# alexmeli100/pbrt-rust

Hardware: AMD Instinct MI355X
Metric: Msamples/s (camera rays x spp) at 1920x1080 (higher is better)
Workload: dtype f32

## Files before the change

include/mi355pt.h:

```cpp
#ifndef MI355PT_H
#define MI355PT_H

#include <stdint.h>

#ifdef __cplusplus
extern "C" {
#endif

typedef enum PtStatus {
    PT_OK = 0,
    PT_ERR_INVALID_ARG = 1,
    PT_ERR_NO_DEVICE = 2,
    PT_ERR_HIP = 3,
    PT_ERR_UNSUPPORTED = 4,
    PT_ERR_SOBOL_DIMENSIONS = 5,
    PT_ERR_STACK_OVERFLOW = 6,
    PT_ERR_OUT_OF_MEMORY = 7,
    PT_ERR_PROBE_CHAIN = 8
} PtStatus;


enum {
    PT_TRI_REVERSE_ORIENTATION = 1u << 0,
    PT_TRI_SWAPS_HANDEDNESS    = 1u << 1,
// ... 257 lines not shown
typedef struct PtCounters {
    uint64_t camera_rays;
    uint64_t intersect_tests;
    uint64_t shadow_tests;
    uint64_t bvh_nodes_visited;
    uint64_t triangle_tests;
    uint64_t sphere_tests;
    uint64_t zero_radiance_paths_num, zero_radiance_paths_den;
    uint64_t path_length_hist[16];
    uint64_t sanitized_nan, sanitized_negative, sanitized_infinite;
    uint64_t film_splats;
    uint64_t wavefront_stages;
    uint64_t reference_asserts;
} PtCounters;

typedef struct PtKernelStat {
    char name[32];
    uint64_t launches;
    double total_ms;
    uint64_t items;
    uint64_t bvh_nodes;
    uint64_t triangle_tests;
    char kernel[48];
} PtKernelStat;

typedef struct pt_scene pt_scene;
typedef struct pt_multi_scene pt_multi_scene;


int pt_init(int device_ordinal);
int pt_device_count(int *n_devices);
const char *pt_last_error(void);
int pt_set_trace_exact(int exact);

int pt_scene_create(const PtSceneDesc *desc, pt_scene **out_scene);
void pt_scene_destroy(pt_scene *scene);

int pt_scene_bvh_info(const pt_scene *scene, uint32_t *n_nodes, uint32_t *n_prims);
int pt_scene_bvh_read(const pt_scene *scene, PtBVHNode *nodes, uint32_t *ordered_prims);

int pt_render(pt_scene *scene, const PtRenderParams *params, float *film_xyzw, int film_is_device);
int pt_render_samples(pt_scene *scene, const PtRenderParams *params, uint32_t first_sample, uint32_t n_samples, float *film_xyzw, int film_is_device);
int pt_pass_size(pt_scene *scene, const PtRenderParams *params, uint32_t *spp_per_pass);

int pt_film_resolve(const float *film_xyzw, uint32_t n_pixels, float scale, float *rgb_out);

int pt_film_resolve_device(pt_scene *scene, const float *film_xyzw_dev, uint32_t n_pixels, float scale, float *rgb_dev, uint8_t *srgb8_dev);
int pt_film_halves_error(pt_scene *scene, const float *film_a_dev, const float *film_b_dev, uint32_t width, uint32_t height,
                         float *tile_error_dev, float *mean_error_host, float *max_tile_error_host);

int pt_tile_grid(const PtRenderParams *params, uint32_t *ntx, uint32_t *nty);
int pt_render_tiles(pt_scene *scene, const PtRenderParams *params, uint32_t first_sample, uint32_t n_samples,
                    const uint32_t *tiles, uint32_t n_tiles, float *film_xyzw, int film_is_device);
int pt_tiles_select(pt_scene *scene, const PtRenderParams *params, const float *tile_error_dev, float threshold,
                    const uint32_t *candidates, uint32_t n_candidates, uint32_t *tiles_out, uint32_t *n_out);

int pt_multi_scene_create(const PtSceneDesc *desc, const int *device_ordinals, uint32_t n_devices, pt_multi_scene **out_scene);
void pt_multi_scene_destroy(pt_multi_scene *scene);
int pt_multi_render(pt_multi_scene *scene, const PtRenderParams *params, float *film_xyzw, int film_is_device);
int pt_multi_render_samples(pt_multi_scene *scene, const PtRenderParams *params, uint32_t first_sample, uint32_t n_samples, float *film_xyzw, int film_is_device);
int pt_multi_get_counters(const pt_multi_scene *scene, PtCounters *out);
int pt_multi_get_kernel_stats(const pt_multi_scene *scene, uint32_t replica, PtKernelStat *out, uint32_t max_entries, uint32_t *n_out);
int pt_multi_get_timing(const pt_multi_scene *scene, double *merge_ms, double *render_ms, double *copy_ms, uint32_t max_replicas);
int pt_multi_get_create_timing(const pt_multi_scene *scene, double *wall_ms, double *replica_ms, uint32_t max_replicas);
enum { PT_PEER_SAME_DEVICE = 0, PT_PEER_ENABLED = 1, PT_PEER_STAGED = 2 };
int pt_multi_get_peer_access(const pt_multi_scene *scene, int *peer, uint32_t max_replicas);
void pt_multi_tile_shard(uint32_t tile_rank, uint32_t tile_world, uint32_t replica, uint32_t n_replicas, uint32_t *rank_out, uint32_t *world_out);

int pt_get_counters(const pt_scene *scene, PtCounters *out);
int pt_get_kernel_stats(const pt_scene *scene, PtKernelStat *out, uint32_t max_entries, uint32_t *n_out);

int pt_trace_closest(pt_scene *scene, uint32_t n, const float *origins, const float *dirs,
                     const float *tmax, uint32_t *out_prim, float *out_t, float *out_b);
int pt_trace_any(pt_scene *scene, uint32_t n, const float *origins, const float *dirs,
                 const float *tmax, uint8_t *out_hit);
int pt_sobol_samples(const int32_t sample_bounds[4], uint32_t n, const int32_t *pixel_xy,
                     const uint32_t *sample_num, uint32_t n_dims, float *out, uint64_t *out_index);
int pt_halton_samples(const int32_t sample_bounds[4], uint32_t sample_at_pixel_center, uint32_t n, const int32_t *pixel_xy,
                      const uint32_t *sample_num, uint32_t n_dims, float *out, uint64_t *out_index);
int pt_camera_rays(const PtRenderParams *params, uint32_t n, const float *camera_samples,
                   float *out_origins, float *out_dirs);
int pt_dist1d_sample(const float *func, uint32_t n, int discrete, uint32_t n_u, const float *u,
                     float *out_x, float *out_pdf, int32_t *out_offset);

#ifdef __cplusplus
}
#endif
#endif
```

pbrt-rust_amd/_abi.py:

```python
import ctypes as C

PT_OK = 0
PT_ERR_INVALID_ARG, PT_ERR_NO_DEVICE, PT_ERR_HIP, PT_ERR_UNSUPPORTED = 1, 2, 3, 4
PT_ERR_SOBOL_DIMENSIONS, PT_ERR_STACK_OVERFLOW, PT_ERR_OUT_OF_MEMORY, PT_ERR_PROBE_CHAIN = 5, 6, 7, 8

PT_TRI_REVERSE_ORIENTATION = 1
PT_TRI_SWAPS_HANDEDNESS = 2
PT_TRI_HAS_N = 4
PT_TRI_HAS_S = 8
PT_TRI_HAS_UV = 16

PT_SHAPE_TRIANGLE, PT_SHAPE_SPHERE = 0, 1
PT_NONE = 0xFFFFFFFF

PT_MAT_MATTE, PT_MAT_MIRROR, PT_MAT_GLASS, PT_MAT_PLASTIC, PT_MAT_METAL, PT_MAT_UBER, PT_MAT_SUBSTRATE, PT_MAT_SUBSURFACE, PT_MAT_TRANSLUCENT, PT_MAT_MIX, PT_MAT_DISNEY = range(11)
(PT_DS_METALLIC, PT_DS_SPECULARTINT, PT_DS_ANISOTROPIC, PT_DS_SHEEN, PT_DS_SHEENTINT, PT_DS_CLEARCOAT, PT_DS_CLEARCOATGLOSS, PT_DS_SPECTRANS,
 PT_DS_FLATNESS, PT_DS_DIFFTRANS) = range(10)
PT_LIGHT_DIFFUSE_AREA, PT_LIGHT_DISTANT, PT_LIGHT_POINT, PT_LIGHT_INFINITE, PT_LIGHT_SPOT = range(5)
PT_LS_UNIFORM, PT_LS_POWER, PT_LS_SPATIAL, PT_LS_SPATIAL_EAGER, PT_LS_SPATIAL_LAZY = range(5)
PT_SPLIT_SAH, PT_SPLIT_HLBVH = range(2)
PT_SAMPLER_SOBOL, PT_SAMPLER_HALTON = range(2)
PT_INTEGRATOR_PATH, PT_INTEGRATOR_VOLPATH = range(2)
PT_QUADRIC_SPHERE, PT_QUADRIC_DISK = range(2)

# ... 74 lines not shown
                ("rhoeff", fp), ("profile_cdf", fp)]


class PtSceneDesc(C.Structure):
    _fields_ = [("n_vertices", u32), ("P", fp), ("N", fp), ("S", fp), ("UV", fp),
                ("n_triangles", u32), ("indices", u32p), ("tri_flags", u8p),
                ("n_spheres", u32), ("spheres", C.POINTER(PtSphere)),
                ("n_prims", u32), ("prim_shape", u32p), ("prim_material", u32p), ("prim_light", u32p),
                ("n_materials", u32), ("materials", C.POINTER(PtMaterial)),
                ("n_lights", u32), ("lights", C.POINTER(PtLight)),
                ("env_width", u32), ("env_height", u32), ("env_texels", fp), ("env_importance", fp), ("env_power_lookup", f32 * 3),
                ("max_node_prims", u32), ("n_nodes", u32), ("nodes", C.POINTER(PtBVHNode)), ("ordered_prims", u32p),
                ("n_objects", u32), ("objects", C.POINTER(PtObject)), ("n_instances", u32), ("instances", C.POINTER(PtInstance)),
                ("n_top", u32), ("top_refs", u32p), ("n_bssrdf_tables", u32), ("bssrdf_tables", C.POINTER(PtBSSRDFTable)),
                ("n_textures", u32), ("textures", C.POINTER(PtTexture)), ("tri_alpha", i32p), ("tri_shadow_alpha", i32p), ("n_images", u32), ("images", C.POINTER(PtImage)), ("ewa_weight_lut", fp), ("n_media", u32), ("media", C.POINTER(PtMedium)), ("prim_medium_inside", u32p), ("prim_medium_outside", u32p), ("split_method", u32)]


class PtRenderParams(C.Structure):
    _fields_ = [("full_resolution", i32 * 2), ("cropped_pixel_bounds", i32 * 4), ("filter_radius", f32 * 2),
                ("filter_table", f32 * 256), ("max_sample_luminance", f32), ("scale", f32),
                ("spp", u32), ("sample_bounds", i32 * 4),
                ("raster_to_camera", f32 * 16), ("camera_to_world", f32 * 16), ("lens_radius", f32),
                ("focal_distance", f32), ("shutter_open", f32), ("shutter_close", f32),
                ("max_depth", u32), ("rr_threshold", f32), ("pixel_bounds", i32 * 4), ("light_strategy", u32),
                ("tile_rank", u32), ("tile_world", u32), ("spp_per_pass", u32), ("profile", u32), ("sampler_type", u32), ("sample_at_pixel_center", u32), ("integrator", u32), ("camera_medium", u32)]


class PtCounters(C.Structure):
    _fields_ = [("camera_rays", u64), ("intersect_tests", u64), ("shadow_tests", u64), ("bvh_nodes_visited", u64),
                ("triangle_tests", u64), ("sphere_tests", u64), ("zero_radiance_paths_num", u64),
                ("zero_radiance_paths_den", u64), ("path_length_hist", u64 * 16), ("sanitized_nan", u64),
                ("sanitized_negative", u64), ("sanitized_infinite", u64), ("film_splats", u64),
                ("wavefront_stages", u64), ("reference_asserts", u64)]

    def as_dict(self):
        d = {}
        for name, _ in self._fields_:
            v = getattr(self, name)
            d[name] = list(v) if hasattr(v, "__len__") else int(v)
        return d


class PtKernelStat(C.Structure):
    _fields_ = [("name", C.c_char * 32), ("launches", u64), ("total_ms", C.c_double), ("items", u64), ("bvh_nodes", u64), ("triangle_tests", u64), ("kernel", C.c_char * 48)]


VP = C.c_void_p
ENTRY_POINTS = {
    "pt_init": (C.c_int, [C.c_int]),
    "pt_last_error": (C.c_char_p, []),
    "pt_scene_create": (C.c_int, [C.POINTER(PtSceneDesc), C.POINTER(VP)]),
    "pt_scene_destroy": (None, [VP]),
    "pt_scene_bvh_info": (C.c_int, [VP, u32p, u32p]),
    "pt_scene_bvh_read": (C.c_int, [VP, C.POINTER(PtBVHNode), u32p]),
    "pt_render": (C.c_int, [VP, C.POINTER(PtRenderParams), VP, C.c_int]),
    "pt_render_samples": (C.c_int, [VP, C.POINTER(PtRenderParams), u32, u32, VP, C.c_int]),
    "pt_pass_size": (C.c_int, [VP, C.POINTER(PtRenderParams), u32p]),
    "pt_tile_grid": (C.c_int, [C.POINTER(PtRenderParams), u32p, u32p]),
    "pt_render_tiles": (C.c_int, [VP, C.POINTER(PtRenderParams), u32, u32, u32p, u32, VP, C.c_int]),
    "pt_tiles_select": (C.c_int, [VP, C.POINTER(PtRenderParams), VP, f32, u32p, u32, u32p, u32p]),
    "pt_film_resolve": (C.c_int, [fp, u32, f32, fp]),
    "pt_film_resolve_device": (C.c_int, [VP, VP, u32, f32, VP, VP]),
    "pt_film_halves_error": (C.c_int, [VP, VP, VP, u32, u32, VP, fp, fp]),
    "pt_device_count": (C.c_int, [C.POINTER(C.c_int)]),
    "pt_set_trace_exact": (C.c_int, [C.c_int]),
    "pt_multi_scene_create": (C.c_int, [C.POINTER(PtSceneDesc), C.POINTER(C.c_int), u32, C.POINTER(VP)]),
    "pt_multi_scene_destroy": (None, [VP]),
    "pt_multi_render": (C.c_int, [VP, C.POINTER(PtRenderParams), VP, C.c_int]),
    "pt_multi_render_samples": (C.c_int, [VP, C.POINTER(PtRenderParams), u32, u32, VP, C.c_int]),
    "pt_multi_get_counters": (C.c_int, [VP, C.POINTER(PtCounters)]),
    "pt_multi_get_kernel_stats": (C.c_int, [VP, u32, C.POINTER(PtKernelStat), u32, u32p]),
    "pt_multi_get_timing": (C.c_int, [VP, C.POINTER(C.c_double), C.POINTER(C.c_double), C.POINTER(C.c_double), u32]),
    "pt_multi_get_peer_access": (C.c_int, [VP, C.POINTER(C.c_int), u32]),
    "pt_multi_get_create_timing": (C.c_int, [VP, C.POINTER(C.c_double), C.POINTER(C.c_double), u32]),
    "pt_multi_tile_shard": (None, [u32, u32, u32, u32, u32p, u32p]),
    "pt_get_counters": (C.c_int, [VP, C.POINTER(PtCounters)]),
    "pt_get_kernel_stats": (C.c_int, [VP, C.POINTER(PtKernelStat), u32, u32p]),
    "pt_trace_closest": (C.c_int, [VP, u32, fp, fp, fp, u32p, fp, fp]),
    "pt_trace_any": (C.c_int, [VP, u32, fp, fp, fp, u8p]),
    "pt_sobol_samples": (C.c_int, [i32p, u32, i32p, u32p, u32, fp, u64p]),
    "pt_halton_samples": (C.c_int, [i32p, u32, u32, i32p, u32p, u32, fp, u64p]),
    "pt_camera_rays": (C.c_int, [C.POINTER(PtRenderParams), u32, fp, fp, fp]),
    "pt_dist1d_sample": (C.c_int, [fp, u32, C.c_int, u32, fp, fp, fp, i32p]),
}


def bind(lib, table=ENTRY_POINTS, strict=True):
    for name, (res, args) in table.items():
        fn = getattr(lib, name, None)
        if fn is None:
            if strict:
                raise AttributeError(f"{name}: symbol declared in " + ("include/mi355pt.h" if table is ENTRY_POINTS else "its C header") + " is missing from the library")
            continue
        fn.restype = res
        fn.argtypes = args
    return lib
```

pbrt-rust_amd/csrc/kern_aux.h:

```cpp
#pragma once
#include "kern_shade_common.h"
#include "kern_film.h"
__global__ __launch_bounds__(256) void k_medium_route(DeviceScene s, RenderConst rc, SobolTables tabs, PathSoA ps, const uint32_t *queue, const uint32_t *count_ptr,
                                                     uint32_t *class_count, uint32_t *c0, uint32_t *c1, uint32_t *c2, uint32_t *c3, uint32_t *c4, uint32_t *c5, uint32_t *error) {
    __shared__ LdsQueue<1024> q0, q1, q2, q3, q4, q5;
    lq_init(q0); lq_init(q1); lq_init(q2); lq_init(q3); lq_init(q4); lq_init(q5);
    __syncthreads();
    const uint32_t count = *count_ptr;
    const uint32_t rounded = (count + 255u) & ~255u;
    for (uint32_t qi = blockIdx.x * blockDim.x + threadIdx.x; qi < rounded; qi += gridDim.x * blockDim.x) {
        const bool valid = qi < count;
        uint32_t pid = 0, cls = (uint32_t)kMissClass;
        if (valid) {
            pid = queue[qi];
            const uint32_t hp = ps.hit_prim(pid);
            cls = class_general((ps.hit_pflags(pid) >> kTpClassShift) & kTpClassMask);
            if (cls == (uint32_t)kSpecClass) cls = 1u;
            const uint32_t med = ps.medium(pid);
            if (med != PT_NONE) {
                uint32_t meta = ps.meta(pid);
                Sampler smp = make_sampler(tabs, nullptr, 0u, ps.sobol_index(pid), meta & 0xffffu, rc.halton.enabled != 0);
                const V3 rd(ps.dx(pid), ps.dy(pid), ps.dz(pid));
                bool sampled; float t;
                RGB w(1.0f);
// ... 25 lines not shown
        lq_flush_nosync(q4, class_count + 4, c4, 256u, false); lq_flush_nosync(q5, class_count + 5, c5, 256u, false);
        __syncthreads();
    }
    lq_flush_nosync(q0, class_count + 0, c0, 0u, true); lq_flush_nosync(q1, class_count + 1, c1, 0u, true);
    lq_flush_nosync(q2, class_count + 2, c2, 0u, true); lq_flush_nosync(q3, class_count + 3, c3, 0u, true);
    lq_flush_nosync(q4, class_count + 4, c4, 0u, true); lq_flush_nosync(q5, class_count + 5, c5, 0u, true);
}

__global__ __launch_bounds__(256) void k_shade_medium(DeviceScene s, RenderConst rc, SobolTables tabs, LightGrid grid, PathSoA ps, ShadeJob job) {
    constexpr uint32_t LDS_DIMS = 56u;
    __shared__ uint32_t s_sobol[LDS_DIMS * kSobolNibWords];
    __shared__ VertexQueues<1024, false, true> s_q;
    __shared__ uint32_t s_hist[16];
    s_q.init();
    hist_init(s_hist);
    PT_PROF_BEGIN
    sobol_stage_lds(s_sobol, tabs.nib, LDS_DIMS, threadIdx.x, blockDim.x);
    __syncthreads();
    const uint32_t count = *job.count;
    const uint32_t rounded = (count + 255u) & ~255u;
    unsigned long long zero_num = 0, n_valid = 0, n_bytes = 0;
    uint32_t n_assert = 0;
    for (uint32_t qi = blockIdx.x * blockDim.x + threadIdx.x; qi < rounded; qi += gridDim.x * blockDim.x) {
        const bool valid = qi < count;
        bool push_ext = false, push_resolve = false, push_shadow = false, push_mis = false, push_self = false;
        int finished_bounces = -1;
        uint32_t pid = 0;
        if (valid) {
            n_valid++;
            pid = job.queue[qi];
            const uint32_t meta = ps.meta(pid);
            uint32_t flags = meta >> 24, bounces = (meta >> 16) & 0xffu;
            Sampler smp = make_sampler(tabs, s_sobol, LDS_DIMS, ps.sobol_index(pid), meta & 0xffffu, rc.halton.enabled != 0);
            RGB L(ps.L_r(pid), ps.L_g(pid), ps.L_b(pid));
            RGB beta(ps.beta_r(pid), ps.beta_g(pid), ps.beta_b(pid));
            const bool stage_b = (flags & PF_STAGE_B) != 0u;
            if (stage_b) smp.load_window();
            if (stage_b && s.has_shells) { if (!vol_chain_step<true>(s, ps, pid, flags, smp, push_shadow, push_mis, n_bytes)) resolve_pending<true, true>(s, ps, pid, flags, L, zero_num, n_assert, n_bytes PT_PROF_PASS, nullptr); }
            else resolve_pending<true, true>(s, ps, pid, flags, L, zero_num, n_assert, n_bytes PT_PROF_PASS, stage_b ? &smp : nullptr);
            flags &= ~(PF_CAMERA_RAY | PF_STAGE_B);
            bool terminated = bounces >= rc.max_depth;
            if (!terminated) {
                if (!stage_b) smp.load_window();
                const V3 ro(ps.ox(pid), ps.oy(pid), ps.oz(pid)), rd(ps.dx(pid), ps.dy(pid), ps.dz(pid));
                const uint32_t med = ps.medium(pid);
                SurfaceInteraction si;
                si.p = ro + rd * ps.hit_t(pid); si.wo = -rd; si.n = V3(0.0f, 0.0f, 0.0f); si.sh_n = V3(0.0f, 0.0f, 0.0f); si.p_error = V3(0.0f, 0.0f, 0.0f);
                IData it; it.p = si.p; it.p_error = V3(0.0f, 0.0f, 0.0f); it.n = V3(0.0f, 0.0f, 0.0f);
                const PhaseBsdf phase{s.media[med].g, si.wo};
                bool defer = false;
                if (!stage_b) {
                    if (!nee_vertex<true, PhaseBsdf, true, true>(s, grid, ps, pid, smp, si, it, phase, beta, flags, push_shadow, push_mis, n_bytes PT_PROF_PASS, MedIface{med, med})) L = L + beta * RGB(0.0f);
                }
                defer = (s.has_grid != 0u || s.has_shells != 0u) && (push_shadow || push_mis);
                if (defer) { flags |= PF_STAGE_B; push_self = true; }
                else {
                V3 wi;
                hg_sample_p(phase.g, si.wo, wi, smp.get_2d());
                flags &= ~PF_SPECULAR;
                if (russian_roulette(rc, smp, beta, ps.etascale(pid), bounces, n_assert)) terminated = true;
                else {
                    bounces += 1;
                    ps.ox(pid) = si.p.x; ps.oy(pid) = si.p.y; ps.oz(pid) = si.p.z;
                    ps.dx(pid) = wi.x; ps.dy(pid) = wi.y; ps.dz(pid) = wi.z;
                    push_ext = true;
                }
                }
            }
            if (terminated) {
                if (flags & (PF_PEND_SHADOW | PF_PEND_MIS)) { flags |= PF_DEAD; push_resolve = true; }
                else finished_bounces = (int)bounces;
            }
            store_vertex(ps, pid, L, beta, smp, bounces, flags, job.error);
        }
        s_q.push(job, pid, push_ext, push_resolve, push_shadow, push_mis, push_self);
        if (finished_bounces >= 0) hist_add(s_hist, (uint32_t)finished_bounces);
        s_q.flush(job, 256u, false);
    }
    s_q.flush(job, 0u, true);
    vertex_epilogue(s_hist, job.counters, &job.counters->shade_items[kMediumClass], &job.counters->shade_bytes[kMediumClass], n_valid, n_bytes, n_assert);
    (void)zero_num;
}

template <bool SPH, bool VOL>
__global__ __launch_bounds__(256, PT_MISS_WAVES) void k_shade_miss(DeviceScene s, RenderConst rc, PathSoA ps, ShadeJob job) {
    __shared__ uint32_t s_hist[16];
    hist_init(s_hist);
    PT_PROF_BEGIN
    __syncthreads();
    const uint32_t count = *job.count;
    unsigned long long zero_num = 0, n_valid = 0, n_bytes = 0;
    uint32_t n_assert = 0;
    for (uint32_t qi = blockIdx.x * blockDim.x + threadIdx.x; qi < count; qi += gridDim.x * blockDim.x) {
        n_valid++;
        n_bytes += 4 + 32 +  16 + 4;
        const uint32_t pid = job.queue[qi];
        float4 *cq = reinterpret_cast<float4 *>(ps.core) + 4 * (size_t)pid;
        const float4 c0 = cq[0], c1 = cq[1];
        const uint32_t meta = __float_as_uint(c1.w);
        uint32_t flags = meta >> 24; const uint32_t bounces = (meta >> 16) & 0xffu;
        RGB L(c0.x, c0.y, c0.z);
        resolve_pending<SPH, VOL>(s, ps, pid, flags, L, zero_num, n_assert, n_bytes PT_PROF_PASS);
        if (!(flags & PF_DEAD) && (bounces == 0 || (flags & PF_SPECULAR)) && s.n_infinite > 0) {
            n_bytes += 32;
            const RGB beta(c1.x, c1.y, c1.z);
            const float4 *rq = reinterpret_cast<const float4 *>(ps.ray) + 2 * (size_t)pid;
            const float4 r0 = rq[0], r1 = rq[1];
            const V3 rd(r0.w, r1.x, r1.y);
            add_escaped_le(s, rd, beta, L);
        }
        cq[0] = make_float4(L.r, L.g, L.b, c0.w);
        ps.meta(pid) = (meta & 0x00ffffffu) | ((flags & ~PF_CAMERA_RAY) << 24);
        hist_add(s_hist, bounces);
    }
    __syncthreads();
    counter_add(&job.counters->zero_num, zero_num);
    vertex_epilogue(s_hist, job.counters, &job.counters->shade_items[kMissClass], &job.counters->shade_bytes[kMissClass], n_valid, n_bytes, n_assert);
    (void)rc;
}

template <bool SPH>
__global__ __launch_bounds__(256, PT_FILM_WAVES) void k_film_final(DeviceScene s, RenderConst rc, PathSoA ps, const float *filter_table, float *film_rgbw, DevCounters *counters) {
    __shared__ uint32_t s_hist[16];
    hist_init(s_hist);
    __syncthreads();
    PT_PROF_BEGIN
    unsigned long long zero_num = 0, n_final = 0, n_bytes = 0;
    uint32_t n_assert = 0;
    film_slot(rc, ps, filter_table, film_rgbw, counters, [&](uint32_t pid, RGB &L) {
        const float4 c1 = reinterpret_cast<const float4 *>(ps.core)[4 * (size_t)pid + 1];
        const uint32_t meta = __float_as_uint(c1.w);
        uint32_t flags = meta >> 24; const uint32_t bounces = (meta >> 16) & 0xffu;
        const bool pend = (flags & (PF_PEND_SHADOW | PF_PEND_MIS)) != 0u;
        const bool escaped = !(flags & (PF_DEAD | PF_FINISHED));
        if (!pend && !escaped) return;
        n_final++; n_bytes += 32 + 4;
        resolve_pending<SPH, false, true>(s, ps, pid, flags, L, zero_num, n_assert, n_bytes PT_PROF_PASS);
        if (escaped && (bounces == 0 || (flags & PF_SPECULAR)) && s.n_infinite > 0) {
            n_bytes += 32;
            const RGB beta(c1.x, c1.y, c1.z);
            const float4 *rq = reinterpret_cast<const float4 *>(ps.ray) + 2 * (size_t)pid;
            const float4 r0 = rq[0], r1 = rq[1];
            const V3 rd(r0.w, r1.x, r1.y);
            add_escaped_le(s, rd, beta, L);
        }
        hist_add(s_hist, bounces);
    });
    __syncthreads();
    counter_add(&counters->zero_num, zero_num);
    vertex_epilogue(s_hist, counters, &counters->shade_items[kMissClass], &counters->shade_bytes[kMissClass], n_final, n_bytes, n_assert);
}
```

pbrt-rust_amd/csrc/kern_decl.h:

```cpp
#pragma once
#include "kern_common.h"

template <int ANY, int MODE, bool PROBE, int QUADK> __global__ void k_trace(DeviceScene s, TraceJob job);
template <int MAXL, int MODE, int DIFF> __global__ void k_shade(DeviceScene s, RenderConst rc, SobolTables tabs, LightGrid grid, PathSoA ps, ShadeJob job);
template <bool SPH, bool VOL> __global__ void k_shade_miss(DeviceScene s, RenderConst rc, PathSoA ps, ShadeJob job);
template <bool SPH, bool VOL> __global__ void k_bssrdf(DeviceScene s, RenderConst rc, SobolTables tabs, LightGrid grid, PathSoA ps, BssrdfJob job);
__global__ void k_medium_route(DeviceScene s, RenderConst rc, SobolTables tabs, PathSoA ps, const uint32_t *queue, const uint32_t *count_ptr,
                               uint32_t *class_count, uint32_t *c0, uint32_t *c1, uint32_t *c2, uint32_t *c3, uint32_t *c4, uint32_t *c5, uint32_t *error);
__global__ void k_shade_medium(DeviceScene s, RenderConst rc, SobolTables tabs, LightGrid grid, PathSoA ps, ShadeJob job);
__global__ void k_build_packets(DeviceScene s, const uint32_t *ordered, uint32_t n_refs, TriPacket *out);
__global__ void k_mark_leaf_ends(TriPacket *leaf, const uint32_t *last_index, uint32_t n);
__global__ void k_light_area(DeviceScene s, const uint32_t *head, float *area, float4 *rec);
template <int NQ, int CAP> __global__ void k_route(DeviceScene s, const uint32_t *queue, const uint32_t *count_ptr, PathSoA ps, uint32_t *class_count, RouteJob rj);
__global__ void k_generate(RenderConst rc, SobolTables tabs, PathSoA ps, uint32_t *q_ext, uint32_t *q_ext_count, DevCounters *counters);
__global__ void k_film(RenderConst rc, PathSoA ps, const float *filter_table, float *film_rgbw, DevCounters *counters);
template <bool SPH> __global__ void k_film_final(DeviceScene s, RenderConst rc, PathSoA ps, const float *filter_table, float *film_rgbw, DevCounters *counters);
__global__ void k_film_finish(const float *film_rgbw, float *film_xyzw, uint32_t npix);
__global__ void k_film_resolve(const float4 *film_xyzw, uint32_t n_pixels, float scale, float *rgb, uint8_t *srgb8, int packed);
__global__ void k_film_halves_error(const float4 *film_a, const float4 *film_b, uint32_t width, uint32_t height, uint32_t ntx, float *tile_sum, float *tile_err);
__global__ void k_film_error_reduce(const float *tile_sum, const float *tile_err, uint32_t n_tiles, float n_pixels, float *out);
__global__ void k_tiles_select(RenderConst rc, const float *tile_err, float threshold, const uint32_t *candidates, uint32_t n_candidates, uint32_t *out);
__global__ void k_film_sum(FilmSumArgs a, float4 *dst, int accumulate, size_t n_quads);
__global__ void k_light_grid_contrib(DeviceScene s, uint32_t nvx, uint32_t nvy, uint32_t nvz, float *func, const uint32_t *cells, size_t n_cells, size_t stride);
__global__ void k_light_grid_finish(uint32_t n_lights, size_t ncell, float *func, float *cdf, float *func_int, const uint32_t *cells, size_t stride, unsigned long long *cell_ptr);
template <bool SPH> __global__ void k_light_touch(DeviceScene s, LightGrid g, PathSoA ps, const uint32_t *queue, const uint32_t *count_ptr, uint32_t kind, uint32_t max_depth, uint32_t *req_flag, uint32_t *req_list, uint32_t *req_count);
__global__ void k_halton_samples(SobolTables tabs, HaltonParams hp, uint32_t n, const int32_t *pixel_xy, const uint32_t *sample_num,
                                 uint32_t n_dims, float *out, uint64_t *out_index);
__global__ void k_sobol_samples(SobolTables tabs, SobolParams sp, uint32_t n, const int32_t *pixel_xy, const uint32_t *sample_num,
                                uint32_t n_dims, float *out, uint64_t *out_index);
__global__ void k_camera_rays(RenderConst rc, uint32_t n, const float *cs, float *out_o, float *out_d);
__global__ void k_dist1d_sample(const float *func, const float *cdf, float func_int, int n, int discrete, uint32_t n_u, const float *u, float *out_x, float *out_pdf, int32_t *out_off);
```

pbrt-rust_amd/csrc/kern_misc.h:

```cpp
#pragma once
#include "kern_common.h"
#include "kern_film.h"
__global__ void k_build_packets(DeviceScene s, const uint32_t *ordered, uint32_t n_refs, TriPacket *out) {
    uint32_t i = blockIdx.x * blockDim.x + threadIdx.x;
    if (i >= n_refs) return;
    uint32_t prim = ordered[i];
    TriPacket p;
    if (prim & PT_TOP_INSTANCE) {
        p.x[0] = p.x[1] = p.x[2] = p.y[0] = p.y[1] = p.y[2] = p.z[0] = p.z[1] = p.z[2] = 0.0f;
        p.prim = PT_NONE; p.shape = prim & ~PT_TOP_INSTANCE; p.flags = TP_INSTANCE;
        out[i] = p;
        return;
    }
    uint32_t shape = s.prim_shape[prim];
    p.prim = prim; p.shape = shape; p.flags = 0;
    const uint32_t mat = s.prim_material[prim];
    const uint32_t hi = ((mat == PT_NONE ? 0u : (uint32_t)s.mat_class[mat]) << kTpClassShift) | ((mat == PT_NONE || mat >= kTpMatNone ? kTpMatNone : mat) << kTpMatShift);
    if ((shape >> 30) == PT_SHAPE_TRIANGLE) {
        uint32_t tri = shape & 0x3fffffffu;
        uint32_t i0 = s.indices[3 * tri], i1 = s.indices[3 * tri + 1], i2 = s.indices[3 * tri + 2];
        V3 p0 = ld3(s.P, i0), p1 = ld3(s.P, i1), p2 = ld3(s.P, i2);
        P2 uv[3]; tri_uvs(s, tri, i0, i1, i2, uv);
        V3 dpdu, dpdv;
        bool ok = tri_partials(p0, p1, p2, uv, dpdu, dpdv);
        p.x[0] = p0.x; p.x[1] = p1.x; p.x[2] = p2.x; p.y[0] = p0.y; p.y[1] = p1.y; p.y[2] = p2.y; p.z[0] = p0.z; p.z[1] = p1.z; p.z[2] = p2.z;
        p.flags = (uint32_t)s.tri_flags[tri] | (ok ? 0u : (uint32_t)TP_BOGUS) | hi;
        if ((s.tri_alpha && s.tri_alpha[tri] >= 0) || (s.tri_shadow_alpha && s.tri_shadow_alpha[tri] >= 0)) p.flags |= TP_ALPHA;
    } else {
        p.x[0] = p.x[1] = p.x[2] = p.y[0] = p.y[1] = p.y[2] = p.z[0] = p.z[1] = p.z[2] = 0.0f;
        p.flags = TP_SPHERE | hi;
    }
    out[i] = p;
}

__global__ void k_mark_leaf_ends(TriPacket *leaf, const uint32_t *last_index, uint32_t n) {
    uint32_t i = blockIdx.x * blockDim.x + threadIdx.x;
    if (i < n) leaf[last_index[i]].flags |= TP_LAST;
}

__global__ void k_light_area(DeviceScene s, const uint32_t *head, float *area, float4 *rec) {
    uint32_t i = blockIdx.x * blockDim.x + threadIdx.x;
    if (i >= s.n_lights) return;
    float a = 0.0f;
    const PtLight &L = s.lights[i];
    float4 r0 = make_float4(0.0f, 0.0f, 0.0f, __uint_as_float(head[i])), r1 = make_float4(0.0f, 0.0f, 0.0f, 0.0f), r2 = r1, r4 = r1, r5 = r1;
    if (L.type == PT_LIGHT_DIFFUSE_AREA) {
        uint32_t shape = s.prim_shape[L.prim];
        if ((shape >> 30) == PT_SHAPE_TRIANGLE) {
            uint32_t tri = shape & 0x3fffffffu;
            const V3 p0 = ld3(s.P, s.indices[3 * tri]), p1 = ld3(s.P, s.indices[3 * tri + 1]), p2 = ld3(s.P, s.indices[3 * tri + 2]);
            a = tri_area(p0, p1, p2);
            const uint32_t fl = s.tri_flags[tri];
            const bool flip = ((fl & PT_TRI_REVERSE_ORIENTATION) != 0) != ((fl & PT_TRI_SWAPS_HANDEDNESS) != 0);
            V3 ns = normalize(cross(p1 - p0, p2 - p0));
            if (!(fl & PT_TRI_HAS_N) && flip) ns = ns * -1.0f;
            V3 np = normalize(cross(p0 - p2, p1 - p2));
            if (flip) np = -np;
            P2 uv[3]; tri_uvs(s, tri, s.indices[3 * tri], s.indices[3 * tri + 1], s.indices[3 * tri + 2], uv);
            V3 dpdu, dpdv;
            const bool degenerate = !tri_partials(p0, p1, p2, uv, dpdu, dpdv);
            r4 = make_float4(ns.x, ns.y, ns.z, 1.0f / a); r5 = make_float4(np.x, np.y, np.z, 0.0f);
            r0 = make_float4(p0.x, p0.y, p0.z, __uint_as_float(fl | kLrecValid | (degenerate ? kLrecDegenerate : 0u) | head[i]));
            r1 = make_float4(p1.x, p1.y, p1.z, __uint_as_float(tri)); r2 = make_float4(p2.x, p2.y, p2.z, a);
        } else {
            const PtSphere &S = s.spheres[shape & 0x3fffffffu];
            a = S.kind == PT_QUADRIC_DISK ? S.phi_max * 0.5f * (S.radius * S.radius - S.inner_radius * S.inner_radius)
                                          : S.phi_max * S.radius * (S.z_max - S.z_min);
        }
    }
    area[i] = a;
    float4 *r = rec + 6 * (size_t)i;
    r[0] = r0; r[1] = r1; r[2] = r2; r[3] = make_float4(L.L[0], L.L[1], L.L[2], __uint_as_float(L.two_sided)); r[4] = r4; r[5] = r5;
}
template <int NQ, int CAP>
__global__ __launch_bounds__(256) void k_route(DeviceScene s, const uint32_t *queue, const uint32_t *count_ptr, PathSoA ps, uint32_t *class_count, RouteJob rj) {
    __shared__ LdsQueue<CAP> q[NQ];
#pragma unroll
    for (int k = 0; k < NQ; ++k) lq_init(q[k]);
    __syncthreads();
    const uint32_t count = *count_ptr;
    const uint32_t rounded = (count + 255u) & ~255u;
    for (uint32_t qi = blockIdx.x * blockDim.x + threadIdx.x; qi < rounded; qi += gridDim.x * blockDim.x) {
        const bool valid = qi < count;
        uint32_t pid = 0, cls = (uint32_t)kMissClass;
        if (valid) {
            pid = queue[qi];
            cls = (ps.hit_pflags(pid) >> kTpClassShift) & kTpClassMask;
        }
        const uint32_t slot = (uint32_t)(rj.slot_map >> (4u * cls)) & 15u;
        if (valid && slot == 15u && cls != rj.drop_cls) atomicMax(rj.error, (uint32_t)PT_ERR_UNSUPPORTED);
#pragma unroll
        for (int k = 0; k < NQ; ++k) if ((uint32_t)k < rj.n_slots) lq_push(q[k], pid, valid && slot == (uint32_t)k);
        __syncthreads();
#pragma unroll
        for (int k = 0; k < NQ; ++k) if ((uint32_t)k < rj.n_slots) lq_flush_nosync(q[k], class_count + rj.cls_of_slot[k], rj.buf[k], 256u, false);
        __syncthreads();
    }
#pragma unroll
    for (int k = 0; k < NQ; ++k) if ((uint32_t)k < rj.n_slots) lq_flush_nosync(q[k], class_count + rj.cls_of_slot[k], rj.buf[k], 0u, true);
}
PT_DEV void camera_ray(const RenderConst &rc, float pfx, float pfy, float time_u, P2 plens_u, V3 &o, V3 &d) {
    V3 pcamera = xf_point(rc.raster_to_camera, V3(pfx, pfy, 0.0f));
    V3 ro(0.0f, 0.0f, 0.0f), rd = normalize(pcamera);
    if (rc.lens_radius > 0.0f) {
        P2 dsk = concentric_sample_disk(plens_u);
        float lx = dsk.x * rc.lens_radius, ly = dsk.y * rc.lens_radius;
        float ft = rc.focal_distance / rd.z;
        V3 pfocus = ro + rd * ft;
        ro = V3(lx, ly, 0.0f);
        rd = normalize(pfocus - ro);
    }
    (void)time_u;
    V3 oerr;
    V3 ow = xf_point_err(rc.camera_to_world, ro, oerr);
    V3 dw = xf_vector(rc.camera_to_world, rd);
    float l2 = length_squared(dw);
    if (l2 > 0.0f) { float dt = dot(vabs(dw), oerr) / l2; ow = ow + dw * dt; }
    o = ow; d = dw;
}

constexpr int kGenPlane = 257;
struct GenStage { float4 core[4 * kGenPlane]; float4 ray[2 * kGenPlane]; uint32_t alive[256]; };
PT_DEV void stage_path(GenStage &g, uint32_t t, float pfx, float pfy, V3 o, V3 d, uint64_t index, uint32_t medium) {
    g.core[0 * kGenPlane + t] = make_float4(0.0f, 0.0f, 0.0f, 1.0f);
    g.core[1 * kGenPlane + t] = make_float4(1.0f, 1.0f, 1.0f, __uint_as_float(5u | (PF_CAMERA_RAY << 24)));
    g.core[2 * kGenPlane + t] = make_float4(__uint_as_float((uint32_t)index), __uint_as_float((uint32_t)(index >> 32)), pfx, pfy);
    g.core[3 * kGenPlane + t] = make_float4(__uint_as_float(medium), __uint_as_float(PT_NONE), 0.0f, 0.0f);
    g.ray[0 * kGenPlane + t] = make_float4(o.x, o.y, o.z, d.x); g.ray[1 * kGenPlane + t] = make_float4(d.y, d.z, 0.0f, 0.0f);
}
PT_DEV void flush_paths(const GenStage &g, const PathSoA &ps, uint32_t pid0, uint32_t t) {
    float4 *core = reinterpret_cast<float4 *>(ps.core) + 4 * (size_t)pid0, *ray = reinterpret_cast<float4 *>(ps.ray) + 2 * (size_t)pid0;
#pragma unroll
    for (uint32_t j = 0; j < 4; ++j) { const uint32_t gq = j * 256u + t, p = gq >> 2, q = gq & 3u; if (g.alive[p]) core[gq] = g.core[q * kGenPlane + p]; }
#pragma unroll
    for (uint32_t j = 0; j < 2; ++j) { const uint32_t gq = j * 256u + t, p = gq >> 1, q = gq & 1u; if (g.alive[p]) ray[gq] = g.ray[q * kGenPlane + p]; }
}

__global__ __launch_bounds__(256) void k_generate(RenderConst rc, SobolTables tabs, PathSoA ps, uint32_t *q_ext, uint32_t *q_ext_count, DevCounters *counters) {
    constexpr uint32_t kVdcNibbles = 13;
    __shared__ uint32_t s_nib[kSobolNibbles * 5 * 16];
    __shared__ uint64_t s_vdc[2 * kVdcNibbles * 16];
    __shared__ LdsQueue<1024> s_q;
    __shared__ GenStage s_gen;
    lq_init(s_q);
    const uint32_t m = (uint32_t)rc.sobol.log2_resolution;
    sobol_stage_lds(s_nib, tabs.nib, 5u, threadIdx.x, blockDim.x);
    if (m > 0) for (uint32_t i = threadIdx.x; i < 2 * kVdcNibbles * 16; i += blockDim.x) {
        const uint32_t which = i / (kVdcNibbles * 16), e = i - which * (kVdcNibbles * 16), j = e >> 4, n = e & 15u;
        const uint64_t *col = (which ? tabs.vdc_inv : tabs.vdc) + (m - 1) * 52 + 4 * j;
        uint64_t v = 0;
        for (uint32_t b = 0; b < 4; ++b) if (n & (1u << b)) v ^= col[b];
        s_vdc[i] = v;
    }
    __syncthreads();
    const uint32_t total = rc.n_pix_slots * rc.s_count;
    const uint32_t stride = gridDim.x * blockDim.x;
    const uint32_t rounded = (total + 255u) & ~255u;
    unsigned long long n_alive = 0;
    for (uint32_t pid = blockIdx.x * blockDim.x + threadIdx.x; pid < rounded; pid += stride) {
        bool alive = false;
        if (pid < total) {
            const uint32_t slot = pid % rc.n_pix_slots, sl = pid / rc.n_pix_slots;
            int32_t px, py;
            if (slot_to_pixel(rc, slot, px, py)) {
                const uint64_t sample = rc.s_begin + sl;
                if (rc.halton.enabled) {
                    const uint64_t index = halton_index_for_sample(rc.halton, px, py, sample);
                    const float fx = halton_sample_dimension(tabs, rc.halton, index, 0u), fy = halton_sample_dimension(tabs, rc.halton, index, 1u);
                    const float pfx = (float)px + fx, pfy = (float)py + fy;
                    const float tm = halton_sample_dimension(tabs, rc.halton, index, 2u);
                    const P2 pl(halton_sample_dimension(tabs, rc.halton, index, 3u), halton_sample_dimension(tabs, rc.halton, index, 4u));
                    V3 o, d;
                    camera_ray(rc, pfx, pfy, tm, pl, o, d);
                    stage_path(s_gen, threadIdx.x, pfx, pfy, o, d, index, rc.volpath ? rc.camera_medium : PT_NONE);
                    alive = true;
                } else {
                uint64_t index = 0;
                if (m != 0) {
                    index = sample << (m << 1);
                    uint64_t delta = 0;
                    for (uint64_t f = sample, j = 0; f != 0; f >>= 4, ++j) delta ^= s_vdc[j * 16 + (f & 15u)];
                    uint64_t b = ((uint64_t)((uint32_t)(px - rc.sobol.sb_min[0]) << m) | (uint64_t)(uint32_t)(py - rc.sobol.sb_min[1])) ^ delta;
// ... 158 lines not shown
```

pbrt-rust_amd/csrc/kern_shade_common.h:

```cpp
#pragma once
#include "kern_common.h"

#ifdef PT_REGION_PROFILE
struct Prof { long long *t; int *r; unsigned long long *acc; };
#define PT_PROF_BEGIN __shared__ long long s_pt[4]; __shared__ int s_pr[4]; __shared__ unsigned long long s_pacc[64]; \
    if (threadIdx.x < 64) s_pacc[threadIdx.x] = 0; \
    if (threadIdx.x < 4) { s_pt[threadIdx.x] = clock64(); s_pr[threadIdx.x] = 15; } \
    Prof prof{s_pt, s_pr, s_pacc};
#define PT_PROF_END(counters) do { PT_T(14); __syncthreads(); \
    if (threadIdx.x < 16) atomicAdd(&(counters)->regions[threadIdx.x], prof.acc[threadIdx.x] + prof.acc[16 + threadIdx.x] + prof.acc[32 + threadIdx.x] + prof.acc[48 + threadIdx.x]); } while (0)
#define PT_T(k) do { if ((int)__lane_id() == __ffsll((unsigned long long)__ballot(1)) - 1) { const long long _n = clock64(); const int _w = threadIdx.x >> 6; \
    prof.acc[_w * 16 + prof.r[_w]] += (unsigned long long)(_n - prof.t[_w]); prof.t[_w] = _n; prof.r[_w] = (k); } } while (0)
#define PT_PROF_ARG , Prof prof
#define PT_PROF_PASS , prof
#else
#define PT_T(k) do {} while (0)
#define PT_PROF_BEGIN
#define PT_PROF_END(counters) do {} while (0)
#define PT_PROF_ARG
#define PT_PROF_PASS
#endif

template <bool SPH, bool VOL = false, bool EARLY = false> PT_DEV void resolve_pending(const DeviceScene &s, const PathSoA &ps, uint32_t pid, uint32_t &flags, RGB &L,
                                                unsigned long long &zero_num, uint32_t &n_assert, unsigned long long &n_bytes PT_PROF_ARG, Sampler *smp = nullptr) {
// ... 44 lines not shown
            }
        }
        if (!lrad.is_black()) {
            RGB f(m3.x, m3.y, m3.z);
            if (VOL && !tr_done) {
                const uint32_t mm = ps.mis_medium(pid);
                if (mm != PT_NONE) Tr = Tr * medium_tr(s.media[mm], mp != PT_NONE ? m3.w : PT_INF, wi);
            }
            Ld = Ld + f * lrad * Tr * m1.z / m1.w;
        }
    }
    RGB nb(n3.x, n3.y, n3.z);
    RGB Ldb = nb * (Ld / n2.w);
    if (!VOL && Ldb.is_black() && !(flags & PF_NEE_UNCOUNTED)) zero_num++;
    if (!VOL && !(flags & PF_NEE_UNCOUNTED) && !(Ldb.y() >= 0.0f)) n_assert++;
    L = L + Ldb;
    flags &= ~(PF_PEND_SHADOW | PF_PEND_MIS | PF_NEE_UNCOUNTED);
}

template <bool SPH> PT_DEV bool vol_chain_step(const DeviceScene &s, const PathSoA &ps, uint32_t pid, uint32_t flags, Sampler &smp, bool &push_shadow, bool &push_mis,
                                              unsigned long long &n_bytes) {
    float4 *nq = reinterpret_cast<float4 *>(ps.nee) + 4 * (size_t)pid;
    float4 *mq = reinterpret_cast<float4 *>(ps.mis) + 4 * (size_t)pid;
    float4 *xq = reinterpret_cast<float4 *>(ps.ext) + 8 * (size_t)pid;
    if ((flags & PF_PEND_SHADOW) && __float_as_uint(nq[1].z) != 1u) {
        const float4 n0 = nq[0], n1 = nq[1], n2 = nq[2], n3 = nq[3], h0 = xq[4], h1 = xq[5];
        n_bytes += 64 + 32;
        const uint32_t prim = __float_as_uint(h0.x), sm = __float_as_uint(n3.w);
        const bool hit = prim != PT_NONE;
        const V3 so(n0.x, n0.y, n0.z), sd(n0.w, n1.x, n1.y);
        RGB A(n2.x, n2.y, n2.z);
        bool ended = true;
        if (hit && s.prim_material[prim] != PT_NONE) A = RGB(0.0f);
        else {
            if (sm != PT_NONE) {
                const float t_seg = hit ? h1.y : 1.0f - kShadowEps;
                A = A * (s.media[sm].type == PT_MEDIUM_GRID ? RGB(grid_tr(s.media[sm], s.grid_aux[sm], so, sd, t_seg, smp)) : medium_tr(s.media[sm], t_seg, sd));
            }
            if (hit) {
                SurfaceInteraction hs;
                fill_hit_pkt<SPH>(s, __float_as_uint(h1.z), SPH ? __float_as_uint(h1.x) : PT_NONE, so, sd, h0.y, h0.z, h0.w, hs);
                IData a; a.p = hs.p; a.p_error = hs.p_error; a.n = hs.n;
                IData b; { const float4 x0 = xq[0], x1 = xq[1], x2 = xq[2]; b.p = V3(x0.x, x0.y, x0.z); b.p_error = V3(x1.x, x1.y, x1.z); b.n = V3(x2.x, x2.y, x2.z); }
                V3 o2, d2; spawn_ray_to(a, b, o2, d2);
                const uint32_t sm2 = medium_toward(surface_iface(s, prim, sm), hs.n, d2);
                nq[0] = make_float4(o2.x, o2.y, o2.z, d2.x); nq[1] = make_float4(d2.y, d2.z, 0.0f, n1.w); nq[3] = make_float4(n3.x, n3.y, n3.z, __uint_as_float(sm2));
                push_shadow = true; ended = false; n_bytes += 48 + 4;
            }
        }
        nq[2] = make_float4(A.r, A.g, A.b, n2.w);
        if (!ended) return true;
        nq[1] = make_float4(n1.x, n1.y, __uint_as_float(1u), n1.w);
    }
    if (flags & PF_PEND_MIS) {
        const float4 m0 = mq[0], m1 = mq[1], m3 = mq[3], h0 = xq[6], h1 = xq[7];
        n_bytes += 64 + 32;
        const uint32_t prim = __float_as_uint(h0.x), mm = ps.mis_medium(pid);
        const bool hit = prim != PT_NONE;
        const V3 mo(m0.x, m0.y, m0.z), wi(m0.w, m1.x, m1.y);
        RGB f(m3.x, m3.y, m3.z);
        if (mm != PT_NONE) f = f * (s.media[mm].type == PT_MEDIUM_GRID ? RGB(grid_tr(s.media[mm], s.grid_aux[mm], mo, wi, hit ? h1.y : PT_INF, smp)) : medium_tr(s.media[mm], hit ? h1.y : PT_INF, wi));
        if (hit && s.prim_material[prim] == PT_NONE) {
            SurfaceInteraction hs;
            fill_hit_pkt<SPH>(s, __float_as_uint(h1.z), SPH ? __float_as_uint(h1.x) : PT_NONE, mo, wi, h0.y, h0.z, h0.w, hs);
            IData a; a.p = hs.p; a.p_error = hs.p_error; a.n = hs.n;
            V3 o2; spawn_ray(a, wi, o2);
            ps.mis_medium(pid) = medium_toward(surface_iface(s, prim, mm), hs.n, wi);
            mq[0] = make_float4(o2.x, o2.y, o2.z, wi.x); mq[3] = make_float4(f.r, f.g, f.b, m3.w);
            push_mis = true; n_bytes += 32 + 4;
            return true;
        }
        mq[2] = h0; mq[3] = make_float4(f.r, f.g, f.b, hit ? h1.y : 0.0f);
        ps.mis_medium(pid) = PT_NONE;
    }
    if (flags & PF_PEND_SHADOW) {
        const float4 n1 = nq[1], n3 = nq[3];
        nq[1] = make_float4(n1.x, n1.y, __uint_as_float(PT_NONE), n1.w); nq[3] = make_float4(n3.x, n3.y, n3.z, __uint_as_float(PT_NONE));
    }
    return false;
}


template <int QCAP, bool PROBE, bool SELF> struct VertexQueues {
    LdsQueue<QCAP> ext, res, sh, mis;
    LdsQueue<PROBE ? QCAP : 1> probe;
    LdsQueue<SELF ? QCAP : 1> self;
    PT_DEV void init() { lq_init(ext); lq_init(res); lq_init(sh); lq_init(mis); lq_init(probe); lq_init(self); }
    template <class Job> PT_DEV void push(const Job &job, uint32_t pid, bool to_ext, bool to_resolve, bool to_shadow, bool to_mis, bool to_self = false, bool to_probe = false) {
        lq_push(ext, pid, to_ext);
        lq_push(res, pid, to_resolve && job.shade_next0 != nullptr);
        lq_push(sh, pid, to_shadow);
        lq_push(mis, pid, to_mis);
        if constexpr (PROBE) if (job.probe_next) lq_push(probe, pid, to_probe);
        if constexpr (SELF) lq_push(self, pid, to_self);
    }
    template <class Job> PT_DEV void flush(const Job &job, uint32_t reserve, bool force) {
        __syncthreads();
        lq_flush_nosync(ext, job.ext_next_count, job.ext_next, reserve, force);
        lq_flush_nosync(res, job.shade_next0_count, job.shade_next0, reserve, force);
        lq_flush_nosync(sh, job.shadow_count, job.shadow, reserve, force);
        lq_flush_nosync(mis, job.mis_count, job.mis, reserve, force);
        if constexpr (PROBE) if (job.probe_next) lq_flush_nosync(probe, job.probe_next_count, job.probe_next, reserve, force);
        if constexpr (SELF) lq_flush_nosync(self, job.self_next_count, job.self_next, reserve, force);
        __syncthreads();
    }
};

PT_DEV bool russian_roulette(const RenderConst &rc, Sampler &smp, RGB &beta, float etascale, uint32_t bounces, uint32_t &n_assert) {
    const RGB rrbeta = beta * etascale;
    if (rrbeta.max_component_value() < rc.rr_threshold && bounces > 3) {
        const float q = maxf(1.0f - rrbeta.max_component_value(), 0.05f);
        if (smp.get_1d() < q) return true;
        beta = beta / (1.0f - q); if (__builtin_isinf(beta.y())) n_assert++;
    }
    return false;
}

PT_DEV uint32_t vertex_meta(const Sampler &smp, uint32_t bounces, uint32_t flags, uint32_t *error) {
    if (smp.overflow) atomicMax(error, (uint32_t)PT_ERR_SOBOL_DIMENSIONS);
    return (smp.dim & 0xffffu) | ((bounces & 0xffu) << 16) | (flags << 24);
}
PT_DEV void store_vertex(const PathSoA &ps, uint32_t pid, RGB L, RGB beta, const Sampler &smp, uint32_t bounces, uint32_t flags, uint32_t *error) {
    const uint32_t meta = vertex_meta(smp, bounces, flags, error);
    ps.L_r(pid) = L.r; ps.L_g(pid) = L.g; ps.L_b(pid) = L.b;
    ps.beta_r(pid) = beta.r; ps.beta_g(pid) = beta.g; ps.beta_b(pid) = beta.b;
    ps.meta(pid) = meta;
}

PT_DEV void add_escaped_le(const DeviceScene &s, V3 rd, RGB beta, RGB &L) {
    for (uint32_t k = 0; k < s.n_infinite; ++k) L = L + light_le_infinite(s, s.infinite_lights[k], rd) * beta;
}

PT_DEV void hist_init(uint32_t *s_hist) { if (threadIdx.x < 16) s_hist[threadIdx.x] = 0; }
PT_DEV void hist_add(uint32_t *s_hist, uint32_t bounces) { atomicAdd(&s_hist[bounces > 15u ? 15u : bounces], 1u); }
PT_DEV void vertex_epilogue(const uint32_t *s_hist, DevCounters *c, unsigned long long *items, unsigned long long *bytes, unsigned long long n_valid, unsigned long long n_bytes,
                            uint32_t n_assert) {
    if (threadIdx.x < 16 && s_hist[threadIdx.x]) atomicAdd(&c->path_len[threadIdx.x], (unsigned long long)s_hist[threadIdx.x]);
    counter_add(&c->ref_asserts, (unsigned long long)n_assert);
    counter_add(&c->stages, n_valid);
    counter_add(items, n_valid);
    counter_add(bytes, n_bytes);
}

template <bool SPH, class B, bool VOL = false, bool MEDIUM = false>
PT_DEV bool nee_vertex(const DeviceScene &s, const LightGrid &grid, const PathSoA &ps, uint32_t pid, Sampler &smp,
                                          const SurfaceInteraction &si, const IData &it, const B &bsdf, RGB beta, uint32_t &flags,
                                          bool &push_shadow, bool &push_mis, unsigned long long &n_bytes PT_PROF_ARG, MedIface mif = MedIface{PT_NONE, PT_NONE}) {
    bool nee_pending = false;
    if (s.n_lights > 0) {
        PT_T(5);
        Dist1D distrib = light_distribution_lookup(grid, s, si.p);
        float choice_pdf = 0.0f;
        const uint32_t li = (uint32_t)dist_sample_discrete(distrib, smp.get_1d(), choice_pdf);
        if (choice_pdf != 0.0f) {
            const P2 ulight = smp.get_2d();
            const P2 uscatt = smp.get_2d();
            const int bf = BSDF_ALL & ~BSDF_SPECULAR;
            V3 wi; float lightpdf = 0.0f, scattpdf = 0.0f; IData p1;
            RGB A(0.0f); V3 sh_o(0.0f, 0.0f, 0.0f), sh_d(0.0f, 0.0f, 0.0f);
            uint32_t sh_medium = PT_NONE;
            PT_T(6);
            uint32_t lhead;
            RGB Li = light_sample_li_rec<SPH>(s, li, it, ulight, wi, lightpdf, p1, lhead);
            PT_T(7);
            const bool delta = head_is_delta(lhead);
            if (lightpdf > 0.0f && !Li.is_black()) {
                RGB f = bsdf.f_pdf(si.wo, wi, bf, scattpdf);
                if (!MEDIUM) f = f * abs_dot(wi, si.sh_n);
                if (!f.is_black()) {
                    V3 so, sd; spawn_ray_to(it, p1, so, sd);
                    if (VOL) {
                        const uint32_t sm = medium_toward(mif, it.n, sd);
                        if (s.has_shells) {
                            sh_medium = sm;
                            float4 *xq = reinterpret_cast<float4 *>(ps.ext) + 8 * (size_t)pid;
                            xq[0] = make_float4(p1.p.x, p1.p.y, p1.p.z, 0.0f); xq[1] = make_float4(p1.p_error.x, p1.p_error.y, p1.p_error.z, 0.0f); xq[2] = make_float4(p1.n.x, p1.n.y, p1.n.z, 0.0f);
                            n_bytes += 48;
                        }
                        else if (sm != PT_NONE && s.media[sm].type == PT_MEDIUM_GRID) sh_medium = sm;
                        else if (sm != PT_NONE) Li = Li * medium_tr(s.media[sm], 1.0f - kShadowEps, sd);
                    }
                    A = delta ? f * Li / lightpdf : f * Li * power_heuristic(lightpdf, scattpdf) / lightpdf;
                    sh_o = so; sh_d = sd;
                    flags |= PF_PEND_SHADOW; push_shadow = true; nee_pending = true; n_bytes += 16 + 4;
// ... 78 lines not shown
```

pbrt-rust_amd/csrc/kern_trace.h:

```cpp
#pragma once
#include "kern_common.h"


#ifdef PT_TRACE_UTIL
#define PT_UTIL_DECL \
    uint32_t u_it1 = 0, u_act1 = 0, u_it2 = 0, u_act2 = 0, u_it3 = 0, u_act3 = 0; \
    uint32_t u_ent = 0, u_rej = 0, u_ihit = 0, u_spill = 0;    \
    unsigned long long u_cxf = 0, u_cmain = 0;    \
    unsigned long long u_cfetch = 0, u_cnode = 0, u_cleaf = 0, u_cpop = 0;    \
    long long u_cm = 0; \
    const unsigned long long u_t0 = wall_clock64(); const long long u_t0c = clock64();
#define PT_UTIL(it, act, pred) do { const unsigned long long m_ = __ballot(pred); if (pred) { act++; it += (lane == (uint32_t)(__ffsll((long long)m_) - 1)); } } while (0)
#define PT_UTIL_COUNT(n, pred) do { if (pred) n++; } while (0)
#define PT_UTIL_CLOCK(var) const long long var = clock64(); u_cm = var
#define PT_UTIL_MARK(acc) do { const long long n_ = clock64(); acc += (unsigned long long)(n_ - u_cm); u_cm = n_; } while (0)
#define PT_UTIL_SINCE(acc, var) acc += (unsigned long long)(clock64() - var)
#define PT_UTIL_EPILOGUE \
    if (blockIdx.x == 0 && threadIdx.x == 0) { job.counters->dbg[0] = job.leaf_quorum; job.counters->dbg[1] = job.refill_min; } \
    if (lane == 0) {    \
        const unsigned long long u_t1 = wall_clock64(); \
        atomicMin(&job.counters->tail[0], u_t0); atomicMax(&job.counters->tail[1], u_t1); atomicAdd(&job.counters->tail[4 + 2 * (job.sub[0].kind & 3)], u_t1 - u_t0); \
    } \
    for (int o = 32; o > 0; o >>= 1) { u_it3 += __shfl_xor(u_it3, o); u_act3 += __shfl_xor(u_act3, o); u_ent += __shfl_xor(u_ent, o); u_rej += __shfl_xor(u_rej, o); u_ihit += __shfl_xor(u_ihit, o); u_spill += __shfl_xor(u_spill, o); } \
    if (lane == 0) { atomicAdd(&job.counters->util2[4], (unsigned long long)u_ent); atomicAdd(&job.counters->util2[5], (unsigned long long)u_rej); atomicAdd(&job.counters->util2[6], (unsigned long long)u_ihit); atomicAdd(&job.counters->util2[7], (unsigned long long)u_spill); } \
    if (lane == 0) { \
        atomicAdd(&job.counters->tail[12], (unsigned long long)u_it3); atomicAdd(&job.counters->tail[13], (unsigned long long)u_act3); \
        atomicAdd(&job.counters->tail[14], u_cxf); atomicAdd(&job.counters->tail[15], u_cmain); \
        atomicAdd(&job.counters->util2[0], u_cfetch); atomicAdd(&job.counters->util2[1], u_cnode); atomicAdd(&job.counters->util2[2], u_cleaf); atomicAdd(&job.counters->util2[3], u_cpop); atomicAdd(&job.counters->tail[2], (unsigned long long)(clock64() - (long long)u_t0c)); \
    } \
    for (int o = 32; o > 0; o >>= 1) { u_it1 += __shfl_xor(u_it1, o); u_act1 += __shfl_xor(u_act1, o); u_it2 += __shfl_xor(u_it2, o); u_act2 += __shfl_xor(u_act2, o); } \
    if (lane == 0) { \
        atomicAdd(&job.counters->regions[4 * (job.sub[0].kind & 3) + 0], (unsigned long long)u_it1); atomicAdd(&job.counters->regions[4 * (job.sub[0].kind & 3) + 1], (unsigned long long)u_act1); \
        atomicAdd(&job.counters->regions[4 * (job.sub[0].kind & 3) + 2], (unsigned long long)u_it2); atomicAdd(&job.counters->regions[4 * (job.sub[0].kind & 3) + 3], (unsigned long long)u_act2); \
    }
#else
#define PT_UTIL_DECL
#define PT_UTIL(it, act, pred) do { } while (0)
#define PT_UTIL_COUNT(n, pred) do { } while (0)
#define PT_UTIL_CLOCK(var) do { } while (0)
#define PT_UTIL_MARK(acc) do { } while (0)
#define PT_UTIL_SINCE(acc, var) do { } while (0)
#define PT_UTIL_EPILOGUE
#endif

template <int MODE, bool PROBE, int QUADK> constexpr int trace_waves() {
    if constexpr (MODE == 0 && !PROBE) return QUADK != 0 ? PT_TRACE_WAVES_QUAD : PT_TRACE_WAVES;
    else if constexpr (MODE == 3 && !PROBE) return QUADK != 0 ? PT_TRACE_WAVES_QUAD_INST : PT_TRACE_WAVES_INST;
    else if constexpr (MODE == 0 && PROBE) return PT_TRACE_WAVES_PROBE;
    else return 1;
}
template <int ANY, int MODE, bool PROBE, int QUADK>
__global__ __launch_bounds__(kTraceBlock, (trace_waves<MODE, PROBE, QUADK>())) void k_trace(DeviceScene s, TraceJob job) {
    static_assert(!(ANY != 0 && PROBE), "probe chains are closest-hit queries");
    constexpr bool QUAD = QUADK != 0, BIG = QUADK == 2;
    constexpr bool MIX = ANY == 2;
    constexpr bool SPH = MODE == 1 || MODE == 2, INST = MODE >= 1, ALPHA = MODE == 2;
    constexpr uint32_t kMaskRef = QUAD ? kRefMaskQuad : kRefMask;
    constexpr int kLds = QUAD ? (INST ? kLdsStackQuadInst : kLdsStackQuad) : (MODE == 0 ? kLdsStack : kLdsStackGeneral);
    constexpr int kMaxS = QUAD ? kMaxStackQuad : kMaxStack;
    __shared__ uint32_t lds_stack[(kTraceBlock / 64) * kLds * 2 * 64];
    constexpr bool kWrayHbm = INST && QUAD;
    __shared__ float lds_wray[(INST && !kWrayHbm) ? (kTraceBlock / 64) * 6 * 64 : 1];
    const uint32_t lane = lane_id();
    const uint32_t wave_in_block = threadIdx.x >> 6;
    typedef __attribute__((address_space(3))) uint32_t lds_u32; typedef __attribute__((address_space(1))) uint32_t glb_u32;
    lds_u32 *stack = (lds_u32 *)lds_stack + wave_in_block * (kLds * 2 * 64) + lane;
    float *wray_l = lds_wray + ((INST && !kWrayHbm) ? wave_in_block * (6 * 64) + lane : 0u);
    glb_u32 *spill = (glb_u32 *)job.spill + (size_t)(blockIdx.x * (kTraceBlock / 64) + wave_in_block) * 64 * kSpillWords + lane;
    typedef __attribute__((address_space(1))) float glb_f32;
    glb_f32 *wray_g = (glb_f32 *)(spill + (2 * kSpillEntries) * 64);
    const uint32_t c0 = *job.sub[0].count, c01 = c0 + (MIX ? *job.sub[1].count : 0u);
    const uint32_t count = c01 + (MIX ? *job.sub[2].count : 0u);
    uint32_t ksel = 0; bool lane_any = ANY == 1;
    __shared__ uint32_t lds_kcnt[MIX ? (kTraceBlock / 64) * 16 : 1];
    uint32_t *kcnt = lds_kcnt + (MIX ? (threadIdx.x >> 6) * 16 : 0u);
    if (MIX && lane_id() < 16u) kcnt[lane_id()] = 0u;
    constexpr int kSubRow = 20;
    __shared__ __attribute__((aligned(16))) uint32_t lds_sub[MIX ? 3 * kSubRow : 4];
    if constexpr (MIX) {
        if (threadIdx.x == 0) {
#pragma unroll
            for (int k = 0; k < 3; ++k) {
                const TraceSub &S = job.sub[k];
                uint32_t *r = lds_sub + k * kSubRow;
                const unsigned long long pq = (unsigned long long)S.queue, pr = (unsigned long long)S.ray, ph = (unsigned long long)S.out_hit, ph2 = (unsigned long long)S.out_hit2,
                                         pw = (unsigned long long)S.out_word, pt = (unsigned long long)S.out_t;
                r[0] = (uint32_t)pq; r[1] = (uint32_t)(pq >> 32); r[2] = (uint32_t)pr; r[3] = (uint32_t)(pr >> 32);
                r[4] = S.ray_stride; r[5] = (S.per_ray_tmax ? 1u : 0u) | (S.any ? 2u : 0u); r[6] = __float_as_uint(S.scalar_tmax); r[7] = k == 0 ? 0u : (k == 1 ? c0 : c01);
                r[8] = (uint32_t)ph; r[9] = (uint32_t)(ph >> 32); r[10] = (uint32_t)ph2; r[11] = (uint32_t)(ph2 >> 32);
                r[12] = (uint32_t)pw; r[13] = (uint32_t)(pw >> 32); r[14] = (uint32_t)pt; r[15] = (uint32_t)(pt >> 32);
                r[16] = S.out_hit_stride; r[17] = S.out_word_stride; r[18] = S.out_t_stride; r[19] = 0u;
            }
        }
        __syncthreads();
    }
    const uint4 *const sub_rows = reinterpret_cast<const uint4 *>(lds_sub);
#define PT_GPTR(T, lo, hi) ((__attribute__((address_space(1))) T *)(((unsigned long long)(hi) << 32) | (unsigned long long)(lo)))
#define PT_SUB(f) (job.sub[0].f)
    const uint4 *wide4 = reinterpret_cast<const uint4 *>(s.wide);
    typedef unsigned int v4u __attribute__((ext_vector_type(4)));
    typedef float f2 __attribute__((ext_vector_type(2)));
    const __amdgpu_buffer_rsrc_t rsrc = __builtin_amdgcn_make_buffer_rsrc(const_cast<QuadNode *>(s.quad), 0, BIG ? 0 : (int)(s.pool_quads << 4), 0x00020000);
    typedef __attribute__((address_space(1))) const v4u gpool_u32;
    gpool_u32 *const gpool = (gpool_u32 *)s.quad;
    const uint4 *leaf4 = reinterpret_cast<const uint4 *>(s.leaf);
    uint32_t n_nodes = 0, n_tris = 0, n_rays = 0, n_sph = 0;
    PT_UTIL_DECL

    enum : uint32_t { ST_IDLE = 0, ST_ENTER = 1, ST_LEAF = 2, ST_DONE = 3, ST_INST = 4, ST_RET = 5, ST_LEAFS = 6 };
    uint32_t state = ST_IDLE;
    constexpr int kChunk = PT_TRACE_CHUNK;
    constexpr bool kTailBites = MODE != 0 && PT_TRACE_TAIL_ROUNDS > 0;
    uint32_t bite = kChunk;
    bool exhausted = false;
    uint32_t chunk_next = 0, chunk_left = 0;
    uint32_t qwin = 0u, win_base = 0xffffffffu;
    uint32_t pid = 0, cur = 0, sp = 0, pending = 0;
    V3 ro, rd, inv_dir;
    TriRay tray; tray.kz = 2; tray.Sx = tray.Sy = tray.Sz = 0.0f;
    V3 rop;
    uint32_t lofs = 0;
#define PT_TRI_RAY() do { tray = tri_ray_setup(rd); rop = tri_permute(ro, tray.kz); const uint32_t kz_ = (uint32_t)tray.kz, kx_ = kz_ == 2u ? 0u : kz_ + 1u, ky_ = kx_ == 2u ? 0u : kx_ + 1u; lofs = (kx_ << 4) | (ky_ << 12) | (kz_ << 20); } while (0)
    bool nx = false, ny = false, nz = false;
    uint32_t sgn3 = 0;
#define PT_SGN3() do { if (QUAD) sgn3 = 3u * ((nx ? 1u : 0u) | (ny ? 2u : 0u) | (nz ? 4u : 0u)); } while (0)
    float t_max = 0.0f;
    uint32_t hit_pkt = PT_NONE; float hit_t = 0.0f, hb0 = 0.0f, hb1 = 0.0f, hb2 = 0.0f;
    uint32_t in_inst = PT_NONE, hit_inst = PT_NONE; float t_max_world = 0.0f; bool inst_hit = false;
    uint32_t xf_arg = 0;
    constexpr uint32_t kMarker = 0xFFC0DEADu;
    uint32_t nfound = 0, seen = 0; bool rewalk = false;
    V3 pr_target(0.0f, 0.0f, 0.0f); uint32_t pr_mat = PT_NONE; float pr_u1n = 0.0f;
    uint32_t cur_med = PT_NONE;
    uint32_t sv_nodes = 0, sv_tris = 0, sv_rays = 0, sv_sph = 0;
    uint4 *ring = PROBE ? job.ring + (size_t)(blockIdx.x * (kTraceBlock / 64) + wave_in_block) * (kProbeRing * 3 * 64) + lane : nullptr;

    auto pop_next = [&]() {
        for (;;) {
            if (!QUAD) { n_nodes += pending; pending = 0; }
            if (sp == 0) { state = ST_DONE; return; }
            sp--;
            const uint32_t se = min(sp, (uint32_t)(kLds - 1));
            uint32_t w0 = stack[(2 * se) * 64], w1 = stack[(2 * se + 1) * 64];
            asm volatile("" : "+v"(w0), "+v"(w1));
            if (sp >= (uint32_t)kLds) { w0 = spill[(2 * (sp - kLds)) * 64]; w1 = spill[(2 * (sp - kLds) + 1) * 64]; }
            if (INST && w1 == kMarker) {
                xf_arg = w0; state = ST_RET;
                return;
            }
            if (!QUAD) { n_nodes++; pending = (w0 >> 25) & 63u; }
            if (__uint_as_float(w1) < t_max) {
                cur = w0 & kMaskRef;
                state = (w0 & kLeafBit) ? ST_LEAF : ST_ENTER;
                return;
            }
        }
    };

    auto push = [&](uint32_t w0, uint32_t w1) {
        if (sp < (uint32_t)kLds) { stack[(2 * sp) * 64] = w0; stack[(2 * sp + 1) * 64] = w1; }
        else {
            spill[(2 * (sp - kLds)) * 64] = w0; spill[(2 * (sp - kLds) + 1) * 64] = w1;
            PT_UTIL_COUNT(u_spill, true);
        }
        sp++;
    };
    const uint32_t root_ref = QUAD ? s.root_ref4 : s.root_ref;

    for (;;) {
        const unsigned long long donem = __ballot(state == ST_DONE || state == ST_IDLE);
        const unsigned long long busy = __ballot(state == ST_ENTER || state == ST_LEAF || state == ST_LEAFS || state == ST_INST || state == ST_RET);
// ... 11 lines not shown
                        const uint32_t hif_packed = (hif.inside & 0xffffu) | (hif.outside << 16);
                        if (packet_material(s, pfl, hprim) == pr_mat) {
                            if (!rewalk) {
                                const uint32_t k = nfound % (uint32_t)kProbeRing;
                                ring[(3 * k + 0) * 64] = make_uint4(hit_pkt, hit_inst, __float_as_uint(hb0), __float_as_uint(hb1));
                                ring[(3 * k + 1) * 64] = make_uint4(__float_as_uint(hb2), __float_as_uint(ro.x), __float_as_uint(ro.y), __float_as_uint(ro.z));
                                ring[(3 * k + 2) * 64] = make_uint4(__float_as_uint(rd.x), __float_as_uint(rd.y), __float_as_uint(rd.z), hif_packed);
                                if (nfound == 0xffffffffu) atomicMax(job.error, (uint32_t)PT_ERR_PROBE_CHAIN); else nfound++;
                            } else {
                                const uint32_t selected = min(f2u32_sat(pr_u1n * (float)nfound), nfound - 1u);
                                if (seen == selected) { finish = true; job.bs.iface(pid) = hif_packed; }
                                seen++;
                            }
                        }
                        if (!finish) {
                            const V3 d = target - si.p;
                            if (d.x == 0.0f && d.y == 0.0f && d.z == 0.0f) chain_end = true;
                            else { ro = offset_ray_origin(si.p, si.p_error, si.n, d); rd = d; next_seg = true; cur_med = medium_toward(hif, si.n, d); }
                        }
                    } else chain_end = true;
                    if (chain_end) {
                        if (!rewalk && nfound > 0u) {
                            const uint32_t selected = min(f2u32_sat(pr_u1n * (float)nfound), nfound - 1u);
                            if (nfound - selected <= (uint32_t)kProbeRing) {
                                const uint32_t k = selected % (uint32_t)kProbeRing;
                                const uint4 e0 = ring[(3 * k + 0) * 64], e1 = ring[(3 * k + 1) * 64], e2 = ring[(3 * k + 2) * 64];
                                hit_pkt = e0.x; hit_inst = e0.y; hb0 = __uint_as_float(e0.z); hb1 = __uint_as_float(e0.w); hb2 = __uint_as_float(e1.x);
                                ro = V3(__uint_as_float(e1.y), __uint_as_float(e1.z), __uint_as_float(e1.w));
                                rd = V3(__uint_as_float(e2.x), __uint_as_float(e2.y), __uint_as_float(e2.z));
                                job.bs.iface(pid) = e2.w;
                                finish = true;
                            } else {
                                rewalk = true; seen = 0u; cur_med = PT_NONE;
                                sv_nodes = n_nodes; sv_tris = n_tris; sv_rays = n_rays; sv_sph = n_sph;
                                { const float4 st = job.bs.probe[(size_t)pid * BssSoA::kProbeQuads]; ro = V3(st.x, st.y, st.z); } rd = target - ro;
                                next_seg = true;
                            }
                        } else { hit_pkt = PT_NONE; finish = true; }
                    }
                    if (next_seg || finish) {
                        float4 *rw = const_cast<float4 *>(job.sub[0].ray) + (size_t)pid * job.sub[0].ray_stride;
                        rw[0] = make_float4(ro.x, ro.y, ro.z, rd.x); rw[1] = make_float4(rd.y, rd.z, 0.0f, 0.0f);
                    }
                    if (next_seg) {
                        retire = false;
                        t_max = job.sub[0].scalar_tmax;
                        inv_dir = V3(1.0f / rd.x, 1.0f / rd.y, 1.0f / rd.z);
                        nx = inv_dir.x < 0.0f; ny = inv_dir.y < 0.0f; nz = inv_dir.z < 0.0f; PT_SGN3();
                        PT_TRI_RAY();
                        sp = 0; pending = 0;
                        hit_pkt = PT_NONE; hit_t = 0.0f; hb0 = hb1 = hb2 = 0.0f;
                        in_inst = PT_NONE; hit_inst = PT_NONE; inst_hit = false;
                        n_rays++;
                        state = ST_DONE;
                        if (s.n_nodes > 0) {
                            if (QUAD && !(root_ref & kLeafBit)) { cur = root_ref & kMaskRef; state = ST_ENTER; }
                            else {
                                n_nodes++;
                                if (slab_test(s.root_min, s.root_max, ro, inv_dir, nx, ny, nz, t_max)) {
                                    cur = root_ref & kMaskRef;
                                    state = (root_ref & kLeafBit) ? ST_LEAF : ST_ENTER;
                                }
                            }
                        }
                    } else {
                        if (rewalk) { n_nodes = sv_nodes; n_tris = sv_tris; n_rays = sv_rays; n_sph = sv_sph; }
                        job.bs.nfound(pid) = nfound;
                    }
                }
            }
            typedef float v4f_ __attribute__((ext_vector_type(4)));
            typedef __attribute__((address_space(1))) v4f_ gf4; typedef __attribute__((address_space(1))) uint32_t gu32; typedef __attribute__((address_space(1))) float gf32;
            typedef __attribute__((address_space(1))) const uint32_t gcu32; typedef __attribute__((address_space(1))) const v4f_ gcf4;
            uint32_t hit_prim = PT_NONE, hit_fl = (uint32_t)kMissClass << kTpClassShift;
            if (retire && !lane_any && hit_pkt != PT_NONE) { hit_prim = s.leaf[hit_pkt].prim; hit_fl = s.leaf[hit_pkt].flags; }
            const uint32_t r_pid = pid, r_ksel = ksel, r_pkt = hit_pkt, r_inst = hit_inst, r_nn = n_nodes, r_nt = n_tris; const bool r_any = lane_any;
            const float r_b0 = hb0, r_b1 = hb1, r_b2 = hb2;
            const float r_t = (INST || PROBE) ? hit_t : (hit_pkt != PT_NONE ? t_max : 0.0f);
            if (retire) state = ST_IDLE;
            bool get = false; v4f_ rr0 = {0.0f, 0.0f, 0.0f, 0.0f}, rr1 = rr0, pb0 = rr0, pb1 = rr0; bool per_ray_tmax = PT_SUB(per_ray_tmax) != 0u; float scalar_tmax = PT_SUB(scalar_tmax);
            auto load_window = [&](uint32_t base, uint32_t left) {
                const uint32_t qi = base + lane; uint32_t w = 0u;
                if (lane < left) {
                    uint32_t qk = qi; gcu32 *qp = (gcu32 *)PT_SUB(queue);
                    if constexpr (MIX) {
                        const uint32_t kk = (qi >= c0 ? 1u : 0u) + (qi >= c01 ? 1u : 0u);
                        const uint4 r0 = sub_rows[5u * kk], r1 = sub_rows[5u * kk + 1u];
                        qp = PT_GPTR(const uint32_t, r0.x, r0.y); qk = qi - r1.w;
                    }
                    w = qp ? qp[qk] : qk;
                }
                return w;
            };
            if (!exhausted) {
                if (chunk_left == 0) {
                    uint32_t base = 0;
                    if (lane == 0) base = atomicAdd(job.head, kTailBites ? bite : (uint32_t)kChunk);
                    chunk_next = __shfl(base, 0);
                    chunk_left = (chunk_next < count) ? min(kTailBites ? bite : (uint32_t)kChunk, count - chunk_next) : 0u;
                    if constexpr (kTailBites) {
                        const uint32_t grid_round = gridDim.x * (kTraceBlock / 64) * (uint32_t)kChunk;
                        const uint32_t behind = count > chunk_next + bite ? count - chunk_next - bite : 0u;
                        bite = behind < grid_round / 4u ? (uint32_t)kChunk / 16u : behind < (uint32_t)PT_TRACE_TAIL_ROUNDS * grid_round ? (uint32_t)kChunk / 4u : (uint32_t)kChunk;
                    }
                    if (chunk_left == 0) exhausted = true;
                }
                if (chunk_left != 0u && win_base != chunk_next) { qwin = load_window(chunk_next, chunk_left); win_base = chunk_next; }
                const unsigned long long idlem = PROBE ? __ballot(state == ST_IDLE) : donem;
                const uint32_t rank = __builtin_amdgcn_mbcnt_hi((uint32_t)(idlem >> 32), __builtin_amdgcn_mbcnt_lo((uint32_t)idlem, 0u));
                const uint32_t take = min(chunk_left, (uint32_t)__popcll(idlem));
                const uint32_t wsel = (uint32_t)__shfl((int)qwin, (int)(rank & 63u));
                const uint32_t qi = chunk_next + rank;
                get = state == ST_IDLE && rank < take;
                chunk_next += take; chunk_left -= take;
                if (get) {
                    gcf4 *rays = (gcf4 *)PT_SUB(ray); uint32_t ray_stride = PT_SUB(ray_stride);
                    pid = wsel;
                    if constexpr (MIX) {
                        ksel = (qi >= c0 ? 1u : 0u) + (qi >= c01 ? 1u : 0u);
                        const uint4 r0 = sub_rows[5u * ksel], r1 = sub_rows[5u * ksel + 1u];
                        rays = PT_GPTR(const v4f_, r0.z, r0.w);
                        ray_stride = r1.x; per_ray_tmax = (r1.y & 1u) != 0u; lane_any = (r1.y & 2u) != 0u; scalar_tmax = __uint_as_float(r1.z);
                    }
                    gcf4 *const rp = rays + (size_t)pid * ray_stride;
                    rr0 = rp[0]; rr1 = rp[1];
                    if constexpr (PROBE) { gcf4 *const pp = (gcf4 *)job.bs.probe + (size_t)pid * BssSoA::kProbeQuads; pb0 = pp[0]; pb1 = pp[1]; }
                }
            }
            asm volatile("" :: "v"(hit_prim), "v"(hit_fl), "v"(rr0), "v"(rr1));
            if constexpr (PROBE) asm volatile("" :: "v"(pb0), "v"(pb1));
            if (retire) {
                gf4 *o_hit = (gf4 *)PT_SUB(out_hit), *o_hit2 = (gf4 *)PT_SUB(out_hit2); gu32 *o_word = (gu32 *)PT_SUB(out_word); gf32 *o_t = (gf32 *)PT_SUB(out_t);
                uint32_t o_hit_stride = PT_SUB(out_hit_stride), o_word_stride = PT_SUB(out_word_stride), o_t_stride = PT_SUB(out_t_stride);
                if constexpr (MIX) {
                    const uint4 r2 = sub_rows[5u * r_ksel + 2u], r3 = sub_rows[5u * r_ksel + 3u], r4 = sub_rows[5u * r_ksel + 4u];
                    o_hit = PT_GPTR(v4f_, r2.x, r2.y); o_hit2 = PT_GPTR(v4f_, r2.z, r2.w); o_word = PT_GPTR(uint32_t, r3.x, r3.y); o_t = PT_GPTR(float, r3.z, r3.w);
                    o_hit_stride = r4.x; o_word_stride = r4.y; o_t_stride = r4.z;
                }
                if (r_any) o_word[(size_t)r_pid * o_word_stride] = r_pkt != PT_NONE ? 1u : 0u;
                else {
                    if (o_hit) o_hit[(size_t)r_pid * o_hit_stride] = v4f_{__uint_as_float(hit_prim), r_b0, r_b1, r_b2};
                    else o_word[(size_t)r_pid * o_word_stride] = hit_prim;
                    if (o_hit2) o_hit2[(size_t)r_pid * o_hit_stride] = v4f_{__uint_as_float(INST ? r_inst : PT_NONE), r_t, __uint_as_float(r_pkt), __uint_as_float(hit_fl)};
                    if (o_t) o_t[(size_t)r_pid * o_t_stride] = r_t;
                }
                if constexpr (MIX) {
                    atomicAdd(&kcnt[3u * r_ksel], r_nn); atomicAdd(&kcnt[3u * r_ksel + 1u], r_nt); atomicAdd(&kcnt[3u * r_ksel + 2u], 1u);
                }
            }
            if (get) {
                if constexpr (MIX) { n_nodes = 0u; n_tris = 0u; }
                ro = V3(rr0.x, rr0.y, rr0.z);
                rd = V3(rr0.w, rr1.x, rr1.y);
                t_max = per_ray_tmax ? rr1.z : scalar_tmax;
                inv_dir = V3(1.0f / rd.x, 1.0f / rd.y, 1.0f / rd.z);
                nx = inv_dir.x < 0.0f; ny = inv_dir.y < 0.0f; nz = inv_dir.z < 0.0f; PT_SGN3();
                PT_TRI_RAY();
                sp = 0; pending = 0;
                hit_pkt = PT_NONE; hit_t = 0.0f; hb0 = hb1 = hb2 = 0.0f;
                in_inst = PT_NONE; hit_inst = PT_NONE; inst_hit = false;
                if (PROBE) { nfound = 0u; seen = 0u; rewalk = false; cur_med = PT_NONE; pr_u1n = pb0.w; pr_target = V3(pb1.x, pb1.y, pb1.z); pr_mat = __float_as_uint(pb1.w); }
                n_rays++;
                state = ST_DONE;
                if (s.n_nodes > 0) {
                    if (QUAD && !(root_ref & kLeafBit)) {
                        cur = root_ref & kMaskRef; state = ST_ENTER;
                    } else {
                        if (!QUAD) n_nodes++;
                        if (slab_test(s.root_min, s.root_max, ro, inv_dir, nx, ny, nz, t_max)) {
                            cur = root_ref & kMaskRef;
                            state = (root_ref & kLeafBit) ? ST_LEAF : ST_ENTER;
                        }
                    }
                }
            }
            if (!exhausted) { if (chunk_left != 0u) { qwin = load_window(chunk_next, chunk_left); win_base = chunk_next; } else win_base = 0xffffffffu; }
        }
        if (__ballot(state != ST_IDLE) == 0ull) break;

        const bool at_node = state == ST_ENTER;
        const unsigned long long leaf_m = __ballot(state == ST_LEAF);
        const bool no_node_lane = __ballot(at_node) == 0ull;
        if (__ballot(state == ST_LEAFS) == 0ull && ((uint32_t)__popcll(leaf_m) >= job.leaf_quorum || (no_node_lane && leaf_m != 0ull))) { if (state == ST_LEAF) state = ST_LEAFS; }
        const bool at_leaf = state == ST_LEAFS;
        if constexpr (INST) {
            const unsigned long long xf_m = __ballot(state == ST_INST || state == ST_RET);
            if (xf_m != 0ull && ((uint32_t)__popcll(xf_m) >= job.inst_quorum || __ballot(at_node || at_leaf) == 0ull)) {
                bool need_pop = false;
                PT_UTIL(u_it3, u_act3, state == ST_INST || state == ST_RET);
                PT_UTIL_CLOCK(u_c0);
                if (state == ST_RET) {
                    const uint32_t w0 = xf_arg;
                    if (!QUAD) pending = (w0 >> 25) & 63u;
                    if constexpr (kWrayHbm) { ro = V3(wray_g[0], wray_g[64], wray_g[128]); rd = V3(wray_g[192], wray_g[256], wray_g[320]); }
                    else { ro = V3(wray_l[0], wray_l[64], wray_l[128]); rd = V3(wray_l[192], wray_l[256], wray_l[320]); }
                    inv_dir = V3(1.0f / rd.x, 1.0f / rd.y, 1.0f / rd.z);
                    nx = inv_dir.x < 0.0f; ny = inv_dir.y < 0.0f; nz = inv_dir.z < 0.0f; PT_SGN3();
                    PT_TRI_RAY();
                    PT_UTIL_COUNT(u_ihit, inst_hit);
                    t_max = inst_hit ? t_max : t_max_world;
                    in_inst = PT_NONE; inst_hit = false;
                    if (w0 & kLeafBit) { cur = w0 & kMaskRef; state = ST_LEAF; }
// ... 226 lines not shown
```

pbrt-rust_amd/csrc/kernels.h:

```cpp
#pragma once
#include "knobs.h"
#include <cstddef>
#include "dev_scene.h"
#include "dev_sampler.h"
#include "dev_light.h"
#include "dev_bssrdf.h"

namespace ptd {

constexpr int kNumClasses = 11;
constexpr int kMissClass = 4, kMediumClass = 5, kSpecClass = 6, kMetalClass = 7, kPlasticClass = 8, kUberClass = 9, kSssClass = 10;
PT_HD uint32_t class_general(uint32_t c) { return c == (uint32_t)kMetalClass ? 1u : c == (uint32_t)kPlasticClass ? 2u : (c == (uint32_t)kUberClass || c == (uint32_t)kSssClass) ? 3u : c; }
constexpr int kRouteSlots = 12;
struct RouteJob { uint32_t n_slots; unsigned long long slot_map; uint32_t cls_of_slot[kRouteSlots]; uint32_t *buf[kRouteSlots]; uint32_t *error; uint32_t drop_cls; };
constexpr int kRouteQueueCap = 2048;
constexpr int kLdsStack = PT_LDS_STACK;
constexpr int kLdsStackGeneral = PT_LDS_STACK_GENERAL;
constexpr int kMaxStack = 64;
constexpr int kLdsStackQuad = PT_LDS_STACK_QUAD;
constexpr int kLdsStackQuadInst = PT_LDS_STACK_QUAD_INST;
constexpr int kMaxStackQuad = 96;
constexpr int kLdsStackMinQuad = kLdsStackQuad < kLdsStackQuadInst ? kLdsStackQuad : kLdsStackQuadInst, kLdsStackMinTwo = kLdsStack < kLdsStackGeneral ? kLdsStack : kLdsStackGeneral;
constexpr int kSpillEntries = (kMaxStackQuad - kLdsStackMinQuad) > (kMaxStack - kLdsStackMinTwo) ? (kMaxStackQuad - kLdsStackMinQuad) : (kMaxStack - kLdsStackMinTwo);
constexpr int kSpillWords = 2 * kSpillEntries + 8;
constexpr int kTraceBlock = 256;
constexpr int kProbeRing = 8;

enum : uint32_t { PF_SPECULAR = 1u, PF_PEND_SHADOW = 2u, PF_PEND_MIS = 4u, PF_DEAD = 8u, PF_NEE_UNCOUNTED = 16u,
                  PF_CAMERA_RAY = 32u,
                  PF_STAGE_B = 64u,
                  PF_FINISHED = 128u };

struct PathSoA {
    float *core, *ray, *hit, *nee, *mis, *ext;
    static constexpr int kCoreWords = 16, kRayWords = 8, kHitWords = 8, kNeeWords = 16, kMisWords = 16, kExtWords = 32;
#define PT_REC_F(name, arr, words, off) PT_HD float &name(size_t p) const { return arr[p * words + off]; }
#define PT_REC_U(name, arr, words, off) PT_HD uint32_t &name(size_t p) const { return reinterpret_cast<uint32_t *>(arr)[p * words + off]; }
    PT_REC_F(L_r, core, 16, 0) PT_REC_F(L_g, core, 16, 1) PT_REC_F(L_b, core, 16, 2) PT_REC_F(etascale, core, 16, 3)
    PT_REC_F(beta_r, core, 16, 4) PT_REC_F(beta_g, core, 16, 5) PT_REC_F(beta_b, core, 16, 6)
    PT_REC_U(meta, core, 16, 7)
    PT_HD uint64_t &sobol_index(size_t p) const { return reinterpret_cast<uint64_t *>(core)[p * 8 + 4]; }
    PT_REC_F(pfilm_x, core, 16, 10) PT_REC_F(pfilm_y, core, 16, 11)
    PT_REC_U(medium, core, 16, 12)
    PT_REC_U(mis_medium, core, 16, 13)
    PT_REC_F(ox, ray, 8, 0) PT_REC_F(oy, ray, 8, 1) PT_REC_F(oz, ray, 8, 2) PT_REC_F(dx, ray, 8, 3) PT_REC_F(dy, ray, 8, 4) PT_REC_F(dz, ray, 8, 5)
    PT_REC_U(hit_prim, hit, 8, 0) PT_REC_F(hit_b0, hit, 8, 1) PT_REC_F(hit_b1, hit, 8, 2) PT_REC_F(hit_b2, hit, 8, 3)
    PT_REC_U(hit_inst, hit, 8, 4)
    PT_REC_F(hit_t, hit, 8, 5)
    PT_REC_U(hit_pkt, hit, 8, 6)
    PT_REC_U(hit_pflags, hit, 8, 7)
    PT_REC_F(sh_ox, nee, 16, 0) PT_REC_F(sh_oy, nee, 16, 1) PT_REC_F(sh_oz, nee, 16, 2) PT_REC_F(sh_dx, nee, 16, 3) PT_REC_F(sh_dy, nee, 16, 4) PT_REC_F(sh_dz, nee, 16, 5)
    PT_REC_U(occluded, nee, 16, 6)
    PT_REC_U(sh_prim, nee, 16, 6)
    PT_REC_U(nee_light, nee, 16, 7)
    PT_REC_F(A_r, nee, 16, 8) PT_REC_F(A_g, nee, 16, 9) PT_REC_F(A_b, nee, 16, 10)
    PT_REC_F(nee_choice_pdf, nee, 16, 11)
    PT_REC_F(nb_r, nee, 16, 12) PT_REC_F(nb_g, nee, 16, 13) PT_REC_F(nb_b, nee, 16, 14)
    PT_REC_F(mis_ox, mis, 16, 0) PT_REC_F(mis_oy, mis, 16, 1) PT_REC_F(mis_oz, mis, 16, 2) PT_REC_F(mis_dx, mis, 16, 3) PT_REC_F(mis_dy, mis, 16, 4) PT_REC_F(mis_dz, mis, 16, 5)
    PT_REC_F(mis_w, mis, 16, 6) PT_REC_F(mis_spdf, mis, 16, 7)
    PT_REC_U(mis_prim, mis, 16, 8) PT_REC_F(mis_b0, mis, 16, 9) PT_REC_F(mis_b1, mis, 16, 10) PT_REC_F(mis_b2, mis, 16, 11)
    PT_REC_F(mis_f_r, mis, 16, 12) PT_REC_F(mis_f_g, mis, 16, 13) PT_REC_F(mis_f_b, mis, 16, 14)
    PT_REC_F(mis_t, mis, 16, 15)
#undef PT_REC_F
#undef PT_REC_U
};
constexpr int kPathBytes = 4 * (PathSoA::kCoreWords + PathSoA::kRayWords + PathSoA::kHitWords + PathSoA::kNeeWords + PathSoA::kMisWords);
struct BssSoA {
    float4 *probe, *frame, *coef;
    static constexpr int kProbeQuads = 2, kFrameQuads = 3, kCoefQuads = 2;
    PT_HD uint32_t &nfound(size_t p) const { return reinterpret_cast<uint32_t *>(frame)[p * 12 + 3]; }
    PT_HD uint32_t &iface(size_t p) const { return reinterpret_cast<uint32_t *>(frame)[p * 12 + 7]; }
};
constexpr int kBssBytes = 16 * (BssSoA::kProbeQuads + BssSoA::kFrameQuads + BssSoA::kCoefQuads);
PT_HD bool bss_coef_stored(uint32_t n_textures, const PtMaterial &m) { return n_textures > 0u || m.kd_subsurface != 0u; }

struct QueueSet {
    uint32_t *ext[2];
    uint32_t *shade[2][kNumClasses];
    uint32_t *shadow, *mis;
    uint32_t *probe[2];
};
struct QCounters {
    uint32_t ext[2];
    uint32_t shade[2][kNumClasses];
    uint32_t shadow, mis;
    uint32_t probe[2];
    uint32_t head[4];
    uint32_t error;
    uint32_t pad;
};

constexpr int kMaxReplicas = 64;
struct FilmSumArgs { const float4 *src[kMaxReplicas]; uint32_t n; };

struct DevCounters {
    unsigned long long camera_rays, intersect_tests, shadow_tests, nodes, tri_tests, sphere_tests;
    unsigned long long zero_num, zero_den, path_len[16], san_nan, san_neg, san_inf, splats, stages;
    unsigned long long ref_asserts;
    unsigned long long shade_items[kNumClasses], shade_bytes[kNumClasses];
    unsigned long long regions[16];
    unsigned long long tail[16];
    unsigned long long util2[8];
    unsigned long long dbg[4];
    unsigned long long bss_items, bss_bytes;
    unsigned long long k_nodes[5], k_tris[5], k_rays[5];
};

struct RenderConst {
    uint32_t n_tile_slots;
    uint32_t tile_rank, tile_world;
    uint32_t ntx, nty;
    uint32_t spp, s_begin, s_count;
    uint32_t n_pix_slots;
    int32_t sample_bounds[4], pixel_bounds[4], crop[4];
    SobolParams sobol;
    HaltonParams halton;
    M4 raster_to_camera, camera_to_world;
    float lens_radius, focal_distance, shutter_open, shutter_close;
    float dx_camera[3], dy_camera[3];
    float inv_sqrt_spp;
    uint32_t max_depth; float rr_threshold;
    uint32_t volpath, camera_medium;
    float filter_radius[2]; float max_sample_luminance;
    uint32_t film_w, film_h;
    const uint32_t *tile_list;
};

struct TraceSub {
    const uint32_t *queue;
    const uint32_t *count;
    const float4 *ray; uint32_t ray_stride; uint32_t per_ray_tmax;
    float scalar_tmax;
    float4 *out_hit; uint32_t out_hit_stride;
    uint32_t *out_word; uint32_t out_word_stride;
    float4 *out_hit2;
    float *out_t; uint32_t out_t_stride;
    uint32_t kind;
    uint32_t any;
};

struct TraceJob {
    TraceSub sub[3];
    uint32_t *head;
    uint32_t *spill;
    uint32_t *error;
    DevCounters *counters;
    uint32_t refill_min;
    uint32_t leaf_quorum;
    uint32_t inst_quorum;
    BssSoA bs;
    uint4 *ring;
};

struct ShadeJob {
    const uint32_t *queue; const uint32_t *count;
    uint32_t *ext_next, *ext_next_count;
    uint32_t *shade_next0, *shade_next0_count;
    uint32_t *shadow, *shadow_count, *mis, *mis_count;
    uint32_t *error;
    DevCounters *counters;
    uint32_t cls;
    uint32_t *self_next, *self_next_count;
    uint32_t *probe_next, *probe_next_count;
    BssSoA bs;
};

struct BssrdfJob {
    const uint32_t *queue; const uint32_t *count;
    uint32_t *ext_next, *ext_next_count;
    uint32_t *shade_next0, *shade_next0_count;
    uint32_t *shadow, *shadow_count, *mis, *mis_count;
    uint32_t *error;
    DevCounters *counters;
    BssSoA bs;
    uint32_t *self_next, *self_next_count;
    uint32_t stage_b;
};

}
```

pbrt-rust_amd/csrc/parity_api.hip:

```cpp
#include "host_common.h"

extern "C" {

static int trace_api(pt_scene *sc, bool any, uint32_t n, const float *o, const float *d, const float *tmax, uint32_t *prim, float *t, float *b, uint8_t *hit) {
    DevTmp scratch;
    if (!sc || !o || !d || !tmax) return fail(PT_ERR_INVALID_ARG, "null argument");
    if (n == 0) return PT_OK;
    if (sc->device != g_device) { int bst = bind_device(sc->device); if (bst) return bst; }
    int st = ensure_workspace(sc, 0, 0);
    if (st) return st;
    std::vector<float> recs(8 * (size_t)n, 0.0f);
    for (uint32_t i = 0; i < n; ++i) {
        float *r = recs.data() + 8 * (size_t)i;
        r[0] = o[3 * (size_t)i]; r[1] = o[3 * (size_t)i + 1]; r[2] = o[3 * (size_t)i + 2];
        r[3] = d[3 * (size_t)i]; r[4] = d[3 * (size_t)i + 1]; r[5] = d[3 * (size_t)i + 2]; r[6] = tmax[i];
    }
    float *din = nullptr, *dout = nullptr, *dt = nullptr; uint32_t *docc = nullptr; uint32_t *dcount = nullptr;
    HIP_TRY(scratch.alloc(&din, recs.size() * 4));
    HIP_TRY(scratch.alloc(&dout, 4 * (size_t)n * 4));
    HIP_TRY(scratch.alloc(&dt, (size_t)n * 4));
    HIP_TRY(scratch.alloc(&docc, (size_t)n * 4));
    HIP_TRY(scratch.alloc(&dcount, 4));
    HIP_TRY(hipMemcpy(din, recs.data(), recs.size() * 4, hipMemcpyHostToDevice));
    HIP_TRY(hipMemcpy(dcount, &n, 4, hipMemcpyHostToDevice));
// ... 38 lines not shown
int pt_trace_any(pt_scene *sc, uint32_t n, const float *o, const float *d, const float *tmax, uint8_t *hit) {
    if (!hit) return fail(PT_ERR_INVALID_ARG, "null output");
    return trace_api(sc, true, n, o, d, tmax, nullptr, nullptr, nullptr, hit);
}

int pt_sobol_samples(const int32_t sb[4], uint32_t n, const int32_t *pixel_xy, const uint32_t *sample_num, uint32_t n_dims, float *out, uint64_t *out_index) {
    DevTmp scratch;
    if (!sb || !pixel_xy || !sample_num || !out) return fail(PT_ERR_INVALID_ARG, "null argument");
    if (n_dims > 1024) return fail(PT_ERR_SOBOL_DIMENSIONS, "SobolSampler can only sample up to 1024 dimensions");
    int st = ensure_device();
    if (st || n == 0) return st;
    PtRenderParams rp{}; std::memcpy(rp.sample_bounds, sb, 16);
    RenderConst rc; fill_render_const(&rp, rc);
    int32_t *dxy; uint32_t *dsn; float *dout; uint64_t *didx;
    HIP_TRY(scratch.alloc(&dxy, (size_t)n * 8)); HIP_TRY(scratch.alloc(&dsn, (size_t)n * 4));
    HIP_TRY(scratch.alloc(&dout, (size_t)n * n_dims * 4 + 4)); HIP_TRY(scratch.alloc(&didx, (size_t)n * 8));
    HIP_TRY(hipMemcpy(dxy, pixel_xy, (size_t)n * 8, hipMemcpyHostToDevice));
    HIP_TRY(hipMemcpy(dsn, sample_num, (size_t)n * 4, hipMemcpyHostToDevice));
    hipLaunchKernelGGL(k_sobol_samples, dim3((n + 255) / 256), dim3(256), 0, 0, g_tabs, rc.sobol, n, dxy, dsn, n_dims, dout, didx);
    HIP_TRY(hipDeviceSynchronize());
    HIP_TRY(hipMemcpy(out, dout, (size_t)n * n_dims * 4, hipMemcpyDeviceToHost));
    if (out_index) HIP_TRY(hipMemcpy(out_index, didx, (size_t)n * 8, hipMemcpyDeviceToHost));
    return PT_OK;
}

int pt_halton_samples(const int32_t sb[4], uint32_t sample_at_pixel_center, uint32_t n, const int32_t *pixel_xy, const uint32_t *sample_num, uint32_t n_dims, float *out, uint64_t *out_index) {
    DevTmp scratch;
    if (!sb || !pixel_xy || !sample_num || !out) return fail(PT_ERR_INVALID_ARG, "null argument");
    if (n_dims > kHaltonMaxDims) return fail(PT_ERR_SOBOL_DIMENSIONS, "HaltonSampler can only sample 1000 dimensions");
    int st = ensure_device();
    if (st || n == 0) return st;
    PtRenderParams rp{}; std::memcpy(rp.sample_bounds, sb, 16); rp.sampler_type = PT_SAMPLER_HALTON; rp.sample_at_pixel_center = sample_at_pixel_center;
    RenderConst rc; fill_render_const(&rp, rc);
    int32_t *dxy; uint32_t *dsn; float *dout; uint64_t *didx;
    HIP_TRY(scratch.alloc(&dxy, (size_t)n * 8)); HIP_TRY(scratch.alloc(&dsn, (size_t)n * 4));
    HIP_TRY(scratch.alloc(&dout, (size_t)n * n_dims * 4 + 4)); HIP_TRY(scratch.alloc(&didx, (size_t)n * 8));
    HIP_TRY(hipMemcpy(dxy, pixel_xy, (size_t)n * 8, hipMemcpyHostToDevice));
    HIP_TRY(hipMemcpy(dsn, sample_num, (size_t)n * 4, hipMemcpyHostToDevice));
    hipLaunchKernelGGL(k_halton_samples, dim3((n + 255) / 256), dim3(256), 0, 0, g_tabs, rc.halton, n, dxy, dsn, n_dims, dout, didx);
    HIP_TRY(hipDeviceSynchronize());
    HIP_TRY(hipMemcpy(out, dout, (size_t)n * n_dims * 4, hipMemcpyDeviceToHost));
    if (out_index) HIP_TRY(hipMemcpy(out_index, didx, (size_t)n * 8, hipMemcpyDeviceToHost));
    return PT_OK;
}

int pt_camera_rays(const PtRenderParams *rp, uint32_t n, const float *cs, float *out_o, float *out_d) {
    DevTmp scratch;
    if (!rp || !cs || !out_o || !out_d) return fail(PT_ERR_INVALID_ARG, "null argument");
    int st = ensure_device();
    if (st || n == 0) return st;
    RenderConst rc; fill_render_const(rp, rc);
    float *dcs, *dout;
    HIP_TRY(scratch.alloc(&dcs, (size_t)n * 20)); HIP_TRY(scratch.alloc(&dout, (size_t)n * 24));
    HIP_TRY(hipMemcpy(dcs, cs, (size_t)n * 20, hipMemcpyHostToDevice));
    hipLaunchKernelGGL(k_camera_rays, dim3((n + 255) / 256), dim3(256), 0, 0, rc, n, dcs, dout, dout + 3 * (size_t)n);
    HIP_TRY(hipDeviceSynchronize());
    HIP_TRY(hipMemcpy(out_o, dout, (size_t)n * 12, hipMemcpyDeviceToHost));
    HIP_TRY(hipMemcpy(out_d, dout + 3 * (size_t)n, (size_t)n * 12, hipMemcpyDeviceToHost));
    return PT_OK;
}

int pt_dist1d_sample(const float *func, uint32_t n, int discrete, uint32_t n_u, const float *u, float *out_x, float *out_pdf, int32_t *out_offset) {
    DevTmp scratch;
    if (!func || !u || !out_x || !out_pdf || !out_offset) return fail(PT_ERR_INVALID_ARG, "null argument");
    if (n == 0) return fail(PT_ERR_INVALID_ARG, "a Distribution1D needs at least one function value");
    int st = ensure_device();
    if (st || n_u == 0) return st;
    std::vector<float> f(func, func + n), cdf; float fint = 0.0f;
    dist1d(f, cdf, fint);
    float *dfunc, *dcdf, *du, *dx, *dpdf; int32_t *doff;
    HIP_TRY(scratch.alloc(&dfunc, (size_t)n * 4)); HIP_TRY(scratch.alloc(&dcdf, ((size_t)n + 1) * 4)); HIP_TRY(scratch.alloc(&du, (size_t)n_u * 4));
    HIP_TRY(scratch.alloc(&dx, (size_t)n_u * 4)); HIP_TRY(scratch.alloc(&dpdf, (size_t)n_u * 4)); HIP_TRY(scratch.alloc(&doff, (size_t)n_u * 4));
    HIP_TRY(hipMemcpy(dfunc, f.data(), (size_t)n * 4, hipMemcpyHostToDevice));
    HIP_TRY(hipMemcpy(dcdf, cdf.data(), ((size_t)n + 1) * 4, hipMemcpyHostToDevice));
    HIP_TRY(hipMemcpy(du, u, (size_t)n_u * 4, hipMemcpyHostToDevice));
    hipLaunchKernelGGL(k_dist1d_sample, dim3((n_u + 255) / 256), dim3(256), 0, 0, dfunc, dcdf, fint, (int)n, discrete, n_u, du, dx, dpdf, doff);
    HIP_TRY(hipDeviceSynchronize());
    HIP_TRY(hipMemcpy(out_x, dx, (size_t)n_u * 4, hipMemcpyDeviceToHost));
    HIP_TRY(hipMemcpy(out_pdf, dpdf, (size_t)n_u * 4, hipMemcpyDeviceToHost));
    HIP_TRY(hipMemcpy(out_offset, doff, (size_t)n_u * 4, hipMemcpyDeviceToHost));
    return PT_OK;
}

}
```

pbrt-rust_amd/csrc/render_loop.hip:

```cpp
#include "host_common.h"
#include <utility>


namespace pth {
#ifdef PT_TRACE_UTIL
__global__ void k_trace_util_fold(DevCounters *dc, uint32_t kind, uint32_t waves, int reset) {
    if (!reset) dc->tail[5 + 2 * kind] += (dc->tail[1] - dc->tail[0]) * waves;
    dc->tail[0] = ~0ull; dc->tail[1] = 0ull;
}
#endif

template <class... P> struct Variant { void (*fn)(P...); std::string name; };
static std::string targ(bool b) { return b ? "true" : "false"; }
static std::string targ(int v) { return std::to_string(v); }
template <class... T> std::string symbol(const char *kernel, T... args) { std::string s = std::string(kernel) + "<", sep; ((s += sep + targ(args), sep = ", "), ...); return s + ">"; }

template <class... P, class... A> void launch(pt_scene *sc, const Variant<P...> &v, dim3 blocks, dim3 threads, const A &...args) { launch(sc, v.name, v.fn, blocks, threads, args...); }
static thread_local uint32_t t_max_blocks = ~0u;
static dim3 blocks_for(uint32_t n_upper, uint32_t per_cu) { return dim3(std::min(std::min<uint32_t>((n_upper + 255) / 256, (uint32_t)g_num_cus * per_cu), t_max_blocks)); }
static bool general_geometry(const pt_scene *sc) { return sc->ds.n_spheres > 0 || sc->ds.n_instances > 0; }

using TraceVariant = Variant<DeviceScene, TraceJob>;
template <int ANY, int MODE, bool PROBE, int QUADK> TraceVariant trace_inst() { return {k_trace<ANY, MODE, PROBE, QUADK>, symbol("k_trace", ANY, MODE, PROBE, QUADK)}; }
template <int... I> const TraceVariant &trace_table(int i, std::integer_sequence<int, I...>) { static const TraceVariant t[] = {trace_inst<I / 12 % 3, I / 3 % 4, I / 12 == 3, I % 3>()...}; return t[i]; }
static const TraceVariant &trace_variant(int any, int mode, bool probe, int quadk) { return trace_table((probe ? 3 : any) * 12 + mode * 3 + quadk, std::make_integer_sequence<int, 48>()); }

using ShadeVariant = Variant<DeviceScene, RenderConst, SobolTables, LightGrid, PathSoA, ShadeJob>;
template <int MAXL, int MODE, int DIFF> const ShadeVariant &shade_inst() {
    constexpr int D = ((MODE == 3 && DIFF >= 2) || (MODE == 2 && DIFF == 6)) ? 0 : DIFF;
    static const ShadeVariant v{k_shade<MAXL, MODE, D>, symbol("k_shade", MAXL, MODE, D)};
    return v;
}
template <int MAXL, int DIFF> const ShadeVariant &shade_variant(int mode) { return mode == 3 ? shade_inst<MAXL, 3, DIFF>() : mode == 2 ? shade_inst<MAXL, 2, DIFF>() : mode == 1 ? shade_inst<MAXL, 1, DIFF>() : shade_inst<MAXL, 0, DIFF>(); }

using MissVariant = Variant<DeviceScene, RenderConst, PathSoA, ShadeJob>;
using BssrdfVariant = Variant<DeviceScene, RenderConst, SobolTables, LightGrid, PathSoA, BssrdfJob>;
template <bool SPH, bool VOL> MissVariant miss_inst() { return {k_shade_miss<SPH, VOL>, symbol("k_shade_miss", SPH, VOL)}; }
template <bool SPH, bool VOL> BssrdfVariant bssrdf_inst() { return {k_bssrdf<SPH, VOL>, symbol("k_bssrdf", SPH, VOL)}; }
static const MissVariant &miss_variant(bool sph, bool vol) { static const MissVariant t[3] = {miss_inst<false, false>(), miss_inst<true, false>(), miss_inst<true, true>()}; return t[vol ? 2 : sph ? 1 : 0]; }
static const BssrdfVariant &bssrdf_variant(bool sph, bool vol) { static const BssrdfVariant t[3] = {bssrdf_inst<false, false>(), bssrdf_inst<true, false>(), bssrdf_inst<true, true>()}; return t[vol ? 2 : sph ? 1 : 0]; }

using FilmFinalVariant = Variant<DeviceScene, RenderConst, PathSoA, const float *, float *, DevCounters *>;
using TouchVariant = Variant<DeviceScene, LightGrid, PathSoA, const uint32_t *, const uint32_t *, uint32_t, uint32_t, uint32_t *, uint32_t *, uint32_t *>;
using RouteVariant = Variant<DeviceScene, const uint32_t *, const uint32_t *, PathSoA, uint32_t *, RouteJob>;
template <bool SPH> FilmFinalVariant film_final_inst() { return {k_film_final<SPH>, symbol("k_film_final", SPH)}; }
template <bool SPH> TouchVariant touch_inst() { return {k_light_touch<SPH>, symbol("k_light_touch", SPH)}; }
template <int NQ, int CAP> RouteVariant route_inst() { return {k_route<NQ, CAP>, symbol("k_route", NQ, CAP)}; }
static const FilmFinalVariant &film_final_variant(bool sph) { static const FilmFinalVariant t[2] = {film_final_inst<false>(), film_final_inst<true>()}; return t[sph]; }
static const TouchVariant &touch_variant(bool sph) { static const TouchVariant t[2] = {touch_inst<false>(), touch_inst<true>()}; return t[sph]; }
static const RouteVariant &route_variant(uint32_t n_slots) { static const RouteVariant t[2] = {route_inst<6, 2048>(), route_inst<12, 1024>()}; return t[n_slots > 6]; }

template <int MAXL, int DIFF> void launch_shade(pt_scene *sc, const RenderConst &rc, const LightGrid &grid, const ShadeJob &job, uint32_t upper) {
    const int mode = rc.volpath ? 3 : sc->ds.n_textures > 0 ? 2 : (general_geometry(sc) || rc.halton.enabled) ? 1 : 0;
    launch(sc, shade_variant<MAXL, DIFF>(mode), blocks_for(upper, PT_SHADE_BLOCKS_PER_CU), dim3(256), sc->ds, rc, g_tabs, grid, sc->ps, job);
}

enum ClassKind { kSurface, kMiss, kMedium, kSpecularOrStageB };
struct ClassInfo { const char *stat; ClassKind kind; void (*launch)(pt_scene *, const RenderConst &, const LightGrid &, const ShadeJob &, uint32_t); };
constexpr ClassInfo kClasses[kNumClasses] = {
    {"shade_matte", kSurface, launch_shade<1, 1>}, {"shade_1lobe", kSurface, launch_shade<1, 0>}, {"shade_2lobe", kSurface, launch_shade<2, 0>}, {"shade_manylobe", kSurface, launch_shade<5, 0>},
    {"shade_miss", kMiss, nullptr}, {"shade_medium", kMedium, nullptr}, {"shade_specular", kSpecularOrStageB, launch_shade<1, 2>},
    {"shade_metal", kSurface, launch_shade<1, 3>}, {"shade_plastic", kSurface, launch_shade<2, 4>}, {"shade_uber", kSurface, launch_shade<5, 5>}, {"shade_sss", kSurface, launch_shade<1, 6>}};

static int shaded_in(const pt_scene *sc, int c, bool volpath) { return !sc->class_used[c] ? -1 : !volpath ? c : c == kSpecClass ? 1 : (int)class_general((uint32_t)c); }
static bool class_launched(const pt_scene *sc, int q, bool volpath) { for (int c = 0; c < kNumClasses; ++c) if (shaded_in(sc, c, volpath) == q) return true; return false; }
static bool class_has_queue(const pt_scene *sc, int c) { return c == 0 || kClasses[c].kind != kSurface || class_launched(sc, c, false) || class_launched(sc, c, true); }
static size_t n_queues(const pt_scene *sc) { size_t n = 2 + 2 + (sc->has_bssrdf ? 2 : 0); for (int c = 0; c < kNumClasses; ++c) n += class_has_queue(sc, c) ? 2 : 0; return n; }

int launch_trace(pt_scene *sc, int any, TraceJob job, uint32_t n_upper, bool probe) {
    if (n_upper == 0) return PT_OK;
    const uint32_t knob = job.sub[0].kind == 4 ? 0 : (job.sub[0].kind & 3);
    job.refill_min = (probe && !g_refill_from_env) ? 24u : g_refill_min[knob]; job.leaf_quorum = g_leaf_quorum[knob];
    if (sc->ds.n_instances > 0 && !g_refill_from_env) job.refill_min = 8;
    const uint32_t waves = (n_upper + 63) / 64, blocks = std::min<uint32_t>((waves + 3) / 4, sc->spill_waves / 4);
    const int mode = (sc->ds.tri_alpha || sc->ds.tri_shadow_alpha) ? 2 : sc->ds.n_spheres > 0 ? 1 : sc->ds.n_instances > 0 ? 3 : 0;
    job.inst_quorum = g_inst_quorum;
    if (sc->quad_walk_only && (g_trace_exact || sc->exact_walk_only)) return fail(PT_ERR_UNSUPPORTED, "the two-wide (exact) walk addresses 2^25 records / packets: this scene has the production walk only");
    const int quadk = (g_trace_exact || sc->exact_walk_only) ? 0 : sc->pool_big ? 2 : 1;
#ifdef PT_TRACE_UTIL
    hipLaunchKernelGGL(k_trace_util_fold, dim3(1), dim3(1), 0, sc->stream, sc->dc, job.sub[0].kind & 3u, 0u, 1);
#endif
    launch(sc, trace_variant(any, mode, probe, quadk), dim3(blocks), dim3(kTraceBlock), sc->ds, job);
#ifdef PT_TRACE_UTIL
    hipLaunchKernelGGL(k_trace_util_fold, dim3(1), dim3(1), 0, sc->stream, sc->dc, job.sub[0].kind & 3u, blocks * (kTraceBlock / 64), 0);
#endif
    HIP_TRY(hipGetLastError());
    return PT_OK;
}

int ensure_workspace(pt_scene *sc, size_t capacity, size_t film_px) {
    if (!sc->stream) HIP_TRY(hipStreamCreate(&sc->stream));
    if (!sc->qc) {
        int st;
        if ((st = sc->dalloc(&sc->qc, 1))) return st;
        if ((st = sc->dalloc(&sc->dc, 1))) return st;
        sc->spill_waves = (uint32_t)g_num_cus * g_trace_waves_per_cu;
        if ((st = sc->dalloc(&sc->spill, (size_t)sc->spill_waves * 64 * kSpillWords))) return st;
        if ((st = sc->dalloc(&sc->d_filter, 256))) return st;
        if (sc->has_bssrdf && (st = sc->dalloc(&sc->probe_ring, (size_t)sc->spill_waves * 64 * kProbeRing * 3))) return st;
    }
    if (capacity > sc->capacity) {
        auto drop = [&]() {
            if (sc->slab) hipFree(sc->slab); if (sc->qbuf) hipFree(sc->qbuf); if (sc->ext_slab) hipFree(sc->ext_slab); if (sc->bss_slab) hipFree(sc->bss_slab);
            sc->slab = nullptr; sc->qbuf = nullptr; sc->ext_slab = nullptr; sc->bss_slab = nullptr; sc->ext_capacity = 0; sc->capacity = 0;
        };
        auto oom = [&](const char *what, hipError_t e) { (void)hipGetLastError(); drop(); return fail(PT_ERR_OUT_OF_MEMORY, std::string(what) + ": " + hipGetErrorString(e)); };
        drop();
        size_t bytes = capacity * (size_t)kPathBytes + 4096;
        hipError_t e = hipMalloc(&sc->slab, bytes);
        if (e != hipSuccess) { sc->slab = nullptr; return oom("path-state slab", e); }
        char *p = (char *)sc->slab;
        PathSoA &ps = sc->ps;
        ps.core = (float *)p; p += capacity * (size_t)PathSoA::kCoreWords * 4;
        ps.nee = (float *)p; p += capacity * (size_t)PathSoA::kNeeWords * 4;
        ps.mis = (float *)p; p += capacity * (size_t)PathSoA::kMisWords * 4;
        ps.ray = (float *)p; p += capacity * (size_t)PathSoA::kRayWords * 4;
        ps.hit = (float *)p; p += capacity * (size_t)PathSoA::kHitWords * 4;
        if (sc->has_bssrdf) {
            e = hipMalloc(&sc->bss_slab, capacity * (size_t)kBssBytes);
            if (e != hipSuccess) { sc->bss_slab = nullptr; return oom("BSSRDF probe state", e); }
            BssSoA &bs = sc->bs;
            float4 *bp = (float4 *)sc->bss_slab;
            bs.probe = bp; bp += capacity * (size_t)BssSoA::kProbeQuads; bs.frame = bp; bp += capacity * (size_t)BssSoA::kFrameQuads; bs.coef = bp;
        }
        e = hipMalloc((void **)&sc->qbuf, n_queues(sc) * capacity * 4);
        if (e != hipSuccess) { sc->qbuf = nullptr; return oom("queues", e); }
        uint32_t *qp = sc->qbuf;
        for (int i = 0; i < 2; ++i) { sc->q.ext[i] = qp; qp += capacity; }
        for (int i = 0; i < 2; ++i) for (int c = 0; c < kNumClasses; ++c) { sc->q.shade[i][c] = nullptr; if (class_has_queue(sc, c)) { sc->q.shade[i][c] = qp; qp += capacity; } }
        sc->q.shadow = qp; qp += capacity; sc->q.mis = qp; qp += capacity;
        sc->q.probe[0] = sc->q.probe[1] = nullptr;
        if (sc->has_bssrdf) { sc->q.probe[0] = qp; qp += capacity; sc->q.probe[1] = qp; }
        sc->capacity = capacity;
    }
    if (film_px > sc->film_px) {
        if (sc->film_rgbw) hipFree(sc->film_rgbw);
        sc->film_rgbw = nullptr; sc->film_px = 0;
        if (hipError_t e = hipMalloc((void **)&sc->film_rgbw, film_px * 16); e != hipSuccess) { (void)hipGetLastError(); sc->film_rgbw = nullptr; return fail(PT_ERR_OUT_OF_MEMORY, std::string("device film: ") + hipGetErrorString(e)); }
        sc->film_px = film_px;
    }
    return PT_OK;
}

void spatial_voxels(const pt_scene *sc, uint32_t nvox[3]) {
    float diag[3] = {sc->ds.wb_max[0] - sc->ds.wb_min[0], sc->ds.wb_max[1] - sc->ds.wb_min[1], sc->ds.wb_max[2] - sc->ds.wb_min[2]};
    int me = (diag[0] > diag[1] && diag[0] > diag[2]) ? 0 : (diag[1] > diag[2] ? 1 : 2);
    float bmax = diag[me];
    for (int i = 0; i < 3; ++i) {
        float v = std::round(diag[i] / bmax * 64.0f);
        uint32_t nv = (v > 0.0f) ? (uint32_t)v : 0u;
        nvox[i] = std::max<uint32_t>(1u, nv);
    }
}
constexpr size_t kEagerGridEntries = (size_t)1 << 25;

static void light_grid_cells(pt_scene *sc, const LightGrid &g, size_t n, float *func, float *cdf, float *fint, const uint32_t *cells, size_t stride, unsigned long long *cell_ptr) {
    const size_t total = n * g.n_lights;
    sc->begin("light_grid", total);
    launch(sc, "k_light_grid_contrib", k_light_grid_contrib, dim3((unsigned)((total + 255) / 256)), dim3(256), sc->ds, g.nvox[0], g.nvox[1], g.nvox[2], func, cells, cells ? n : 0, stride);
    hipLaunchKernelGGL(k_light_grid_finish, dim3((unsigned)((n + 255) / 256)), dim3(256), 0, sc->stream, g.n_lights, n, func, cdf, fint, cells, stride, cell_ptr);
    sc->end();
}

int ensure_light_grid(pt_scene *sc, int requested, int &effective) {
    effective = requested;
    if (requested == PT_LS_UNIFORM || sc->n_lights == 1) effective = PT_LS_UNIFORM;
    if (requested > PT_LS_SPATIAL_LAZY) effective = PT_LS_SPATIAL;
    if (effective == PT_LS_SPATIAL) {
        uint32_t nv[3]; spatial_voxels(sc, nv);
        effective = (size_t)nv[0] * nv[1] * nv[2] * std::max(1u, sc->n_lights) <= kEagerGridEntries ? PT_LS_SPATIAL_EAGER : PT_LS_SPATIAL_LAZY;
    }
    LightGrid &g = sc->grid[effective];
    if (sc->grid_ready[effective]) return PT_OK;
    g.strategy = effective >= PT_LS_SPATIAL ? (int)PT_LS_SPATIAL : effective; g.n_lights = sc->n_lights; g.nvox[0] = g.nvox[1] = g.nvox[2] = 1;
    g.cell_ptr = nullptr; g.zero_block = 0; g.missing = nullptr;
    const uint32_t nl = sc->n_lights;
    if (nl == 0) { g.strategy = PT_LS_UNIFORM; g.func = g.cdf = g.func_int = nullptr; sc->grid_ready[effective] = true; return PT_OK; }
    if (effective == PT_LS_UNIFORM || effective == PT_LS_POWER) {
        std::vector<float> func(nl, 1.0f), cdf; float fi;
        if (effective == PT_LS_POWER) {
            std::vector<float> area(nl);
            HIP_TRY(hipMemcpy(area.data(), sc->ds.light_area, nl * sizeof(float), hipMemcpyDeviceToHost));
            const float wr = sc->ds.world_radius;
            for (uint32_t i = 0; i < nl; ++i) {
                const PtLight &L = sc->host_lights[i];
                RGB c(L.L[0], L.L[1], L.L[2]), p(0.0f);
                switch (L.type) {
                case PT_LIGHT_DIFFUSE_AREA: p = c * area[i] * kPi; break;
                case PT_LIGHT_DISTANT: p = c * kPi * wr * wr; break;
                case PT_LIGHT_POINT: p = c * 4.0f * kPi; break;
                case PT_LIGHT_SPOT: p = c * 2.0f * kPi * (1.0f - 0.5f * (L.cos_falloff_start + L.cos_total_width)); break;
                case PT_LIGHT_INFINITE: {
                    p = RGB(sc->env_texel0[0], sc->env_texel0[1], sc->env_texel0[2]) * wr * wr * kPi; break;
                }
                default: break;
                }
                func[i] = p.y();
            }
        }
        dist1d(func, cdf, fi);
        int st;
        if ((st = sc->upload(&g.func, func.data(), nl))) return st;
        if ((st = sc->upload(&g.cdf, cdf.data(), nl + 1))) return st;
        if ((st = sc->upload(&g.func_int, &fi, 1))) return st;
    } else if (effective == PT_LS_SPATIAL_LAZY) {
        spatial_voxels(sc, g.nvox);
        pt_scene::LazyGrid &z = sc->lazy;
        z.ncell = (size_t)g.nvox[0] * g.nvox[1] * g.nvox[2];
        z.stride = ((size_t)4 + nl + nl + 1 + 3) & ~(size_t)3;
        int st;
        if ((st = sc->dalloc(&z.cell_ptr, z.ncell))) return st;
        if ((st = sc->dalloc(&z.zero_block, z.stride))) return st;
        if ((st = sc->dalloc(&z.req_flag, z.ncell))) return st;
// ... 1 lines not shown
        if ((st = sc->dalloc(&z.req_count, 2))) return st;
        z.missing = z.req_count + 1;
        HIP_TRY(hipMemset(z.zero_block, 0, z.stride * 4));
        HIP_TRY(hipMemset(z.req_flag, 0, z.ncell * 4));
        HIP_TRY(hipMemset(z.req_count, 0, 8));
        std::vector<unsigned long long> init(z.ncell, (unsigned long long)z.zero_block);
        HIP_TRY(hipMemcpy(z.cell_ptr, init.data(), z.ncell * 8, hipMemcpyHostToDevice));
        g.func = g.cdf = g.func_int = nullptr;
        g.cell_ptr = z.cell_ptr; g.zero_block = (unsigned long long)z.zero_block; g.missing = z.missing;
    } else {
        spatial_voxels(sc, g.nvox);
        size_t ncell = (size_t)g.nvox[0] * g.nvox[1] * g.nvox[2];
        if (ncell * nl > ((size_t)1 << 31)) return fail(PT_ERR_UNSUPPORTED, "PT_LS_SPATIAL_EAGER: voxels x lights > 2^31 (PT_LS_SPATIAL picks the first-touch form for such scenes)");
        float *func, *cdf, *fint; int st;
        if ((st = sc->dalloc(&func, ncell * nl))) return st;
        if ((st = sc->dalloc(&cdf, ncell * (nl + 1)))) return st;
        if ((st = sc->dalloc(&fint, ncell))) return st;
        light_grid_cells(sc, g, ncell, func, cdf, fint, nullptr, 0, nullptr);
        HIP_TRY(hipGetLastError());
        g.func = func; g.cdf = cdf; g.func_int = fint;
    }
    sc->grid_ready[effective] = true;
    return PT_OK;
}

void tile_grid(const PtRenderParams *rp, uint32_t *ntx, uint32_t *nty) {
    const int32_t dx = rp->sample_bounds[2] - rp->sample_bounds[0], dy = rp->sample_bounds[3] - rp->sample_bounds[1];
    *ntx = (uint32_t)((dx + 15) / 16); *nty = (uint32_t)((dy + 15) / 16);
}

void fill_render_const(const PtRenderParams *rp, RenderConst &rc) {
    std::memset(&rc, 0, sizeof rc);
    std::memcpy(rc.sample_bounds, rp->sample_bounds, 16);
    std::memcpy(rc.pixel_bounds, rp->pixel_bounds, 16);
    std::memcpy(rc.crop, rp->cropped_pixel_bounds, 16);
    int32_t dx = rp->sample_bounds[2] - rp->sample_bounds[0], dy = rp->sample_bounds[3] - rp->sample_bounds[1];
    tile_grid(rp, &rc.ntx, &rc.nty);
    int32_t v = std::max(dx, dy); v--; v |= v >> 1; v |= v >> 2; v |= v >> 4; v |= v >> 8; v |= v >> 16; v++;
    rc.sobol.resolution = v; rc.sobol.log2_resolution = 31 - __builtin_clz((uint32_t)v);
    rc.sobol.sb_min[0] = rp->sample_bounds[0]; rc.sobol.sb_min[1] = rp->sample_bounds[1];
    if (rp->sampler_type == PT_SAMPLER_HALTON) {
        rc.halton.enabled = 1; rc.halton.at_center = rp->sample_at_pixel_center ? 1u : 0u;
        const int32_t res[2] = {dx, dy};
        for (int i = 0; i < 2; ++i) {
            const uint32_t base = i == 0 ? 2u : 3u;
            uint32_t scale = 1, e = 0;
            while ((int64_t)scale < (int64_t)std::min(res[i], 128)) { scale *= base; e++; }
            rc.halton.base_scale[i] = scale; rc.halton.base_exp[i] = e;
        }
        rc.halton.stride = rc.halton.base_scale[0] * rc.halton.base_scale[1];
        auto mult_inverse = [](int64_t a, int64_t n) {
            int64_t x0 = 1, x1 = 0, aa = a, bb = n;
            while (bb != 0) { const int64_t q = aa / bb; int64_t t = aa - q * bb; aa = bb; bb = t; t = x0 - q * x1; x0 = x1; x1 = t; }
            return ((x0 % n) + n) % n;
        };
        rc.halton.mult_inv[0] = (uint32_t)mult_inverse(rc.halton.base_scale[1], rc.halton.base_scale[0]);
        rc.halton.mult_inv[1] = (uint32_t)mult_inverse(rc.halton.base_scale[0], rc.halton.base_scale[1]);
    }
    std::memcpy(rc.raster_to_camera.m, rp->raster_to_camera, 64);
    std::memcpy(rc.camera_to_world.m, rp->camera_to_world, 64);
    rc.lens_radius = rp->lens_radius; rc.focal_distance = rp->focal_distance;
    {
        const V3 p2t = xf_point(rc.raster_to_camera, V3(0.0f, 0.0f, 0.0f));
        const V3 dx = xf_point(rc.raster_to_camera, V3(1.0f, 0.0f, 0.0f)) - p2t, dy = xf_point(rc.raster_to_camera, V3(0.0f, 1.0f, 0.0f)) - p2t;
        rc.dx_camera[0] = dx.x; rc.dx_camera[1] = dx.y; rc.dx_camera[2] = dx.z;
        rc.dy_camera[0] = dy.x; rc.dy_camera[1] = dy.y; rc.dy_camera[2] = dy.z;
        rc.inv_sqrt_spp = 1.0f / std::sqrt((float)rp->spp);
    }
    rc.shutter_open = rp->shutter_open; rc.shutter_close = rp->shutter_close;
    rc.max_depth = rp->max_depth; rc.rr_threshold = rp->rr_threshold;
    rc.volpath = rp->integrator == PT_INTEGRATOR_VOLPATH ? 1u : 0u; rc.camera_medium = rc.volpath ? rp->camera_medium : PT_NONE;
    rc.filter_radius[0] = rp->filter_radius[0]; rc.filter_radius[1] = rp->filter_radius[1];
    rc.max_sample_luminance = rp->max_sample_luminance;
    rc.film_w = (uint32_t)(rp->cropped_pixel_bounds[2] - rp->cropped_pixel_bounds[0]);
    rc.film_h = (uint32_t)(rp->cropped_pixel_bounds[3] - rp->cropped_pixel_bounds[1]);
    rc.spp = rp->spp;
    rc.tile_world = rp->tile_world ? rp->tile_world : 1; rc.tile_rank = rp->tile_rank;
}

__global__ void k_reset(QCounters *qc, uint32_t mask, int cur) {
    if (threadIdx.x != 0 || blockIdx.x != 0) return;
    int nxt = 1 - cur;
    if (mask & 1u) { qc->ext[nxt] = 0; qc->probe[nxt] = 0; for (int c = 0; c < kNumClasses; ++c) qc->shade[nxt][c] = 0; }
    if (mask & 2u) { qc->shadow = 0; qc->mis = 0; }
    if (mask & 4u) { for (int i = 0; i < 4; ++i) qc->head[i] = 0; }
    if (mask & 8u) { qc->ext[cur] = 0; qc->probe[cur] = 0; for (int c = 0; c < kNumClasses; ++c) qc->shade[cur][c] = 0; }
}

constexpr size_t kPassMaxPaths = (size_t)1 << PT_PASS_MAX_PATHS_LOG2;
constexpr double kPassMemFraction = 0.65;
uint32_t choose_pass_size(const pt_scene *sc, uint32_t n_pix_slots, uint32_t spp, uint32_t share, bool volpath) {
    const size_t per_path = (size_t)kPathBytes + 4u * n_queues(sc) + (sc->has_bssrdf ? (size_t)kBssBytes : 0u)
                            + ((volpath && sc->has_null_material) ? 4u * (size_t)PathSoA::kExtWords : 0u);
    size_t free_b = 0, total_b = 0;
    if (hipMemGetInfo(&free_b, &total_b) != hipSuccess) { (void)hipGetLastError(); free_b = 0; }
    const size_t afford = std::max(sc->capacity, (size_t)((double)(free_b / std::max(1u, share) + sc->capacity * per_path) * kPassMemFraction) / per_path);
    const size_t paths = std::min(afford, kPassMaxPaths / std::max(1u, share));
    uint32_t S = (uint32_t)std::min<size_t>(spp, std::max<size_t>(1, paths / std::max(1u, n_pix_slots)));
    const uint32_t n_pass = (spp + S - 1) / S;
    return (spp + n_pass - 1) / n_pass;
}

int lazy_light_touch(pt_scene *sc, const RenderConst &rc, const LightGrid &grid, const uint32_t *queue, const uint32_t *count, uint32_t n_upper, uint32_t kind) {
    const pt_scene::LazyGrid &z = sc->lazy;
    if (!grid.cell_ptr || n_upper == 0) return PT_OK;
    sc->begin("light_touch", n_upper);
    launch(sc, touch_variant(general_geometry(sc)), blocks_for(n_upper, 16u), dim3(256), sc->ds, grid, sc->ps, queue, count, kind, rc.max_depth, z.req_flag, z.req_list, z.req_count);
    sc->end();
    return PT_OK;
}
int lazy_light_fill(pt_scene *sc, const LightGrid &grid) {
    if (!grid.cell_ptr) return PT_OK;
    pt_scene::LazyGrid &z = sc->lazy;
    uint32_t n_new = 0;
    HIP_TRY(hipMemcpyAsync(&n_new, z.req_count, 4, hipMemcpyDeviceToHost, sc->stream));
    HIP_TRY(hipStreamSynchronize(sc->stream));
    if (n_new == 0) return PT_OK;
    if (n_new > z.ncell) return fail(PT_ERR_HIP, "light grid: more voxels requested than the grid holds");
    const uint32_t nl = grid.n_lights;
    const size_t per_batch = std::max<size_t>(1, std::min<size_t>(((size_t)1 << 31) / std::max(1u, nl), ((size_t)1 << 28) / z.stride));
    for (size_t first = 0; first < n_new; first += per_batch) {
        const size_t n = std::min<size_t>(per_batch, n_new - first);
        const size_t need = n * z.stride;
        if (need > z.arena_left) {
            const size_t slab = std::max<size_t>(need, (size_t)16 << 20);
            if (int st = sc->dalloc(&z.arena, slab)) return st;
            z.arena_left = slab;
        }
        float *blocks = z.arena; z.arena += need; z.arena_left -= need;
        light_grid_cells(sc, grid, n, blocks, nullptr, nullptr, z.req_list + first, z.stride, z.cell_ptr);
    }
    HIP_TRY(hipMemsetAsync(z.req_count, 0, 4, sc->stream));
    HIP_TRY(hipGetLastError());
    z.filled += n_new;
    return PT_OK;
}

const char *device_error_text(uint32_t code) {
    switch (code) {
    case PT_ERR_STACK_OVERFLOW: return "BVH traversal stack overflow: a ray needed more than 96 pending entries in the four-wide production walk / 64 in the two-wide exact walk (the reference's 64-entry stack, accelerators/bvh.rs:722, has no check)";
    case PT_ERR_PROBE_CHAIN: return "BSSRDF probe chain with more than 2^32 - 1 intersections";
    case PT_ERR_SOBOL_DIMENSIONS: return "a path asked for sampler dimension >= 1024 (Sobol') / 1000 (Halton): the reference panics there (samplers/sobol.rs:69-73)";
    case PT_ERR_UNSUPPORTED: return "a hit's material class has no shade queue in this render (internal: k_route)";
    default: return "error raised on the device";
    }
}
int sync_queue_counters(pt_scene *sc, QCounters &h) {
    HIP_TRY(hipMemcpyAsync(&h, sc->qc, sizeof h, hipMemcpyDeviceToHost, sc->stream));
    HIP_TRY(hipStreamSynchronize(sc->stream));
    if (h.error) return fail((int)h.error, device_error_text(h.error));
    return PT_OK;
}

struct Iter { pt_scene *sc; const RenderConst &rc; const LightGrid &grid; bool fin, profile_exact; int index, cur; uint32_t n_ext, n_resolve, n_shadow, n_mis, n_probe, n_stage_b; };

template <class Job> Job shading_job(const Iter &it, const uint32_t *queue, const uint32_t *count, int self) {
    pt_scene *sc = it.sc; QCounters *qc = sc->qc; const int nxt = 1 - it.cur;
    Job j{}; j.queue = queue; j.count = count;
    j.ext_next = sc->q.ext[nxt]; j.ext_next_count = &qc->ext[nxt];
    if (!it.fin) { j.shade_next0 = sc->q.shade[nxt][kMissClass]; j.shade_next0_count = &qc->shade[nxt][kMissClass]; }
    j.self_next = sc->q.shade[nxt][self]; j.self_next_count = &qc->shade[nxt][self];
    j.shadow = sc->q.shadow; j.shadow_count = &qc->shadow; j.mis = sc->q.mis; j.mis_count = &qc->mis;
    j.error = &qc->error; j.counters = sc->dc;
    return j;
}

static TraceSub trace_sub(uint32_t *queue, uint32_t *count, const float *ray, int ray_words, float tmax, uint32_t kind) {
    TraceSub s{}; s.queue = queue; s.count = count; s.ray = (const float4 *)ray; s.ray_stride = ray_words / 4; s.scalar_tmax = tmax; s.kind = kind; return s;
}
static TraceJob trace_job(pt_scene *sc, int head) { TraceJob tj{}; tj.spill = sc->spill; tj.error = &sc->qc->error; tj.counters = sc->dc; tj.head = &sc->qc->head[head]; return tj; }
static int traced(pt_scene *sc, const char *stat, int any, const TraceJob &tj, uint32_t n_upper, bool probe = false) {
    if (n_upper == 0) return PT_OK;
    sc->begin(stat, n_upper); const int st = launch_trace(sc, any, tj, n_upper, probe); sc->end();
    return st;
}

static int trace_rays(const Iter &it) {
    pt_scene *sc = it.sc; QCounters *qc = sc->qc; PathSoA &ps = sc->ps; const RenderConst &rc = it.rc;
    TraceSub ext = trace_sub(sc->q.ext[it.cur], &qc->ext[it.cur], ps.ray, PathSoA::kRayWords, INFINITY, it.index == 0 ? 3 : 0);
    ext.out_hit = (float4 *)ps.hit; ext.out_hit_stride = PathSoA::kHitWords / 4; ext.out_hit2 = (float4 *)ps.hit + 1;
    TraceSub mis = trace_sub(sc->q.mis, &qc->mis, ps.mis, PathSoA::kMisWords, INFINITY, 1);
    mis.out_hit = (float4 *)&ps.mis_prim(0); mis.out_hit_stride = PathSoA::kMisWords / 4;
    mis.out_t = rc.volpath ? &ps.mis_t(0) : nullptr; mis.out_t_stride = PathSoA::kMisWords;
    const bool shells = rc.volpath && ps.ext != nullptr;
    if (shells) { mis.out_hit = (float4 *)ps.ext + 6; mis.out_hit_stride = PathSoA::kExtWords / 4; mis.out_hit2 = (float4 *)ps.ext + 7; mis.out_t = nullptr; }
    TraceSub sh = trace_sub(sc->q.shadow, &qc->shadow, ps.nee, PathSoA::kNeeWords, 1.0f - 0.0001f, 2);
    sh.out_word = &ps.occluded(0); sh.out_word_stride = PathSoA::kNeeWords; sh.any = rc.volpath ? 0u : 1u;
    if (shells) { sh.out_hit = (float4 *)ps.ext + 4; sh.out_hit_stride = PathSoA::kExtWords / 4; sh.out_hit2 = (float4 *)ps.ext + 5; }
    if (it.n_mis + it.n_shadow == 0 || g_trace_split) {
        auto one = [&](const char *stat, const TraceSub &sub, int head, int any, uint32_t n) { TraceJob tj = trace_job(sc, head); tj.sub[0] = sub; return traced(sc, stat, any, tj, n); };
        int st;
        if ((st = one(it.index == 0 ? "extend_camera" : "extend", ext, 0, 0, it.n_ext)) || (st = one("extend_mis", mis, 1, 0, it.n_mis))) return st;
        return one("shadow", sh, 2, (int)sh.any, it.n_shadow);
    }
    TraceJob tj = trace_job(sc, 0);
    tj.sub[0] = ext; tj.sub[1] = mis; tj.sub[2] = sh;
    return traced(sc, "trace", 2, tj, it.n_ext + it.n_mis + it.n_shadow);
}

static void route_hits(const Iter &it) {
    pt_scene *sc = it.sc; QCounters *qc = sc->qc; const int cur = it.cur;
    if (it.n_ext == 0) return;
    sc->begin("route", it.n_ext);
    if (it.rc.volpath) {
        launch(sc, "k_medium_route", k_medium_route, blocks_for(it.n_ext, 8u), dim3(256), sc->ds, it.rc, g_tabs, sc->ps, sc->q.ext[cur], &qc->ext[cur], &qc->shade[cur][0],
               sc->q.shade[cur][0], sc->q.shade[cur][1], sc->q.shade[cur][2], sc->q.shade[cur][3], sc->q.shade[cur][4], sc->q.shade[cur][5], &qc->error);
    } else {
        RouteJob rj{}; rj.slot_map = ~0ull; rj.error = &qc->error; rj.drop_cls = it.fin ? (uint32_t)kMissClass : ~0u;
        int slot_of[kNumClasses]; std::fill(slot_of, slot_of + kNumClasses, -1);
        for (int c = 0; c < kNumClasses; ++c) {
            const int q = kClasses[c].kind == kMedium ? -1 : kClasses[c].kind == kMiss ? (it.fin ? -1 : c) : shaded_in(sc, c, false);
            if (q < 0) continue;
            if (slot_of[q] < 0) { slot_of[q] = (int)rj.n_slots; rj.cls_of_slot[rj.n_slots] = (uint32_t)q; rj.buf[rj.n_slots++] = sc->q.shade[cur][q]; }
            rj.slot_map = (rj.slot_map & ~(15ull << (4 * c))) | ((unsigned long long)slot_of[q] << (4 * c));
        }
        launch(sc, route_variant(rj.n_slots), blocks_for(it.n_ext, PT_ROUTE_BLOCKS_PER_CU), dim3(256), sc->ds, sc->q.ext[cur], &qc->ext[cur], sc->ps, &qc->shade[cur][0], rj);
    }
    sc->end();
}

static int touch_voxels(const Iter &it) {
    pt_scene *sc = it.sc;
    for (int c = 0; c < kNumClasses; ++c) {
        if (kClasses[c].kind == kMiss || !class_has_queue(sc, c)) continue;
        if (int st = lazy_light_touch(sc, it.rc, it.grid, sc->q.shade[it.cur][c], &sc->qc->shade[it.cur][c], it.n_ext + it.n_resolve + it.n_stage_b, kClasses[c].kind == kMedium ? 1u : 0u)) return st;
    }
    return lazy_light_fill(sc, it.grid);
}

static int probe_chains(const Iter &it) {
    pt_scene *sc = it.sc; QCounters *qc = sc->qc; PathSoA &ps = sc->ps; const int cur = it.cur;
    if (it.n_probe == 0) return PT_OK;
    TraceSub pr = trace_sub(sc->q.probe[cur], &qc->probe[cur], ps.ray, PathSoA::kRayWords, 1.0f - 0.0001f, 4);
    pr.out_hit = (float4 *)ps.hit; pr.out_hit_stride = PathSoA::kHitWords / 4; pr.out_hit2 = (float4 *)ps.hit + 1;
    TraceJob tj = trace_job(sc, 3); tj.sub[0] = pr; tj.bs = sc->bs; tj.ring = sc->probe_ring;
    int st;
    if ((st = traced(sc, "extend_probe", 0, tj, it.n_probe, true))) return st;
    if ((st = lazy_light_touch(sc, it.rc, it.grid, sc->q.probe[cur], &qc->probe[cur], it.n_probe, 2u)) || (st = lazy_light_fill(sc, it.grid))) return st;
    BssrdfJob bj = shading_job<BssrdfJob>(it, sc->q.probe[cur], &qc->probe[cur], kSpecClass);
    bj.bs = sc->bs;
    sc->begin("bssrdf", it.n_probe);
    launch(sc, bssrdf_variant(general_geometry(sc), it.rc.volpath), blocks_for(it.n_probe, PT_SHADE_BLOCKS_PER_CU), dim3(256), sc->ds, it.rc, g_tabs, it.grid, ps, bj);
    sc->end();
    return PT_OK;
}

static void shade_class(const Iter &it, int c, uint32_t n) {
    pt_scene *sc = it.sc; QCounters *qc = sc->qc; const RenderConst &rc = it.rc; const ClassInfo &ci = kClasses[c];
    if (n == 0) return;
    if (ci.kind == kSpecularOrStageB && rc.volpath) {
        if (!sc->has_bssrdf || !(sc->ds.has_grid || sc->ds.has_shells)) return;
        BssrdfJob bj = shading_job<BssrdfJob>(it, sc->q.shade[it.cur][c], &qc->shade[it.cur][c], c);
        bj.bs = sc->bs; bj.stage_b = 1u;
        sc->begin("bssrdf_stage_b", it.profile_exact ? n : 0);
        launch(sc, bssrdf_variant(general_geometry(sc), true), blocks_for(n, PT_SHADE_BLOCKS_PER_CU), dim3(256), sc->ds, rc, g_tabs, it.grid, sc->ps, bj);
        sc->end();
        return;
    }
    if (!class_launched(sc, c, rc.volpath != 0) || (ci.kind == kMiss && it.fin)) return;
    ShadeJob sj = shading_job<ShadeJob>(it, sc->q.shade[it.cur][c], &qc->shade[it.cur][c], c);
    sj.cls = (uint32_t)c;
    if ((c == 3 || c == kSssClass) && sc->has_bssrdf) { sj.probe_next = sc->q.probe[1 - it.cur]; sj.probe_next_count = &qc->probe[1 - it.cur]; sj.bs = sc->bs; }
    sc->begin(ci.stat, it.profile_exact ? n : 0);
    if (ci.kind == kMedium) launch(sc, "k_shade_medium", k_shade_medium, blocks_for(n, 8u), dim3(256), sc->ds, rc, g_tabs, it.grid, sc->ps, sj);
    else if (ci.kind == kMiss) launch(sc, miss_variant(general_geometry(sc), rc.volpath != 0), blocks_for(n, PT_MISS_BLOCKS_PER_CU), dim3(256), sc->ds, rc, sc->ps, sj);
    else ci.launch(sc, rc, it.grid, sj, n);
    sc->end();
}

static int run_pass(pt_scene *sc, RenderConst &rc, const LightGrid &grid, bool rp_profile_exact, int max_iterations) {
    const uint32_t total = rc.n_pix_slots * rc.s_count;
    QCounters *qc = sc->qc;
    Iter it{sc, rc, grid, g_film_final && !rc.volpath, rp_profile_exact};
    const bool debug_iter = getenv("PT_DEBUG_ITER") != nullptr;
    auto reset = [&](uint32_t mask) { hipLaunchKernelGGL(k_reset, dim3(1), dim3(64), 0, sc->stream, qc, mask, it.cur); };
    int st;
    for (it.index = 0, it.cur = 0; it.index <= max_iterations; ++it.index, it.cur = 1 - it.cur) {
        QCounters h;
        if ((st = sync_queue_counters(sc, h))) return st;
        if (it.index == max_iterations) return fail(PT_ERR_PROBE_CHAIN, "pass did not finish within " + std::to_string(max_iterations) + " wavefront iterations");
        const int cur = it.cur;
        if (debug_iter && it.index > 0 && it.index % 2048 == 0) {
            fprintf(stderr, "[iter %d] ext %u shadow %u mis %u probe %u shade:", it.index, h.ext[cur], h.shadow, h.mis, h.probe[cur]);
            for (int c = 0; c < kNumClasses; ++c) fprintf(stderr, " %u", h.shade[cur][c]);
            fprintf(stderr, "\n");
        }
        it.n_ext = h.ext[cur]; it.n_resolve = h.shade[cur][kMissClass]; it.n_shadow = h.shadow; it.n_mis = h.mis; it.n_probe = h.probe[cur];
        it.n_stage_b = 0;
        if (rc.volpath && (sc->ds.has_grid || sc->ds.has_shells)) for (int c = 0; c < kNumClasses; ++c) if (c != kMissClass) it.n_stage_b += h.shade[cur][c];
        if (it.n_ext == 0 && it.n_resolve == 0 && it.n_probe == 0 && it.n_stage_b == 0 && (!it.fin || (it.n_shadow == 0 && it.n_mis == 0))) break;
        reset(4u | 1u);
        if ((st = trace_rays(it))) return st;
        route_hits(it);
        reset(2u);
        if ((st = touch_voxels(it)) || (st = probe_chains(it))) return st;
        uint32_t class_n[kNumClasses];
        if (rp_profile_exact) {
            QCounters h2;
            HIP_TRY(hipMemcpyAsync(&h2, qc, sizeof h2, hipMemcpyDeviceToHost, sc->stream));
            HIP_TRY(hipStreamSynchronize(sc->stream));
            for (int c = 0; c < kNumClasses; ++c) class_n[c] = h2.shade[cur][c];
        } else for (int c = 0; c < kNumClasses; ++c) class_n[c] = it.n_ext + it.n_resolve + it.n_stage_b;
        for (int c = 0; c < kNumClasses; ++c) shade_class(it, c, class_n[c]);
        HIP_TRY(hipGetLastError());
        reset(8u);
    }
    sc->begin("film", total);
    const dim3 fgrid((unsigned)(((size_t)rc.n_pix_slots + 255) / 256));
    if (it.fin) launch(sc, film_final_variant(general_geometry(sc)), fgrid, dim3(256), sc->ds, rc, sc->ps, sc->d_filter, sc->film_rgbw, sc->dc);
    else launch(sc, "k_film", k_film, fgrid, dim3(256), rc, sc->ps, sc->d_filter, sc->film_rgbw, sc->dc);
    sc->end();
    HIP_TRY(hipGetLastError());
    return PT_OK;
}

void read_counters(pt_scene *sc) {
    DevCounters d;
    hipMemcpy(&d, sc->dc, sizeof d, hipMemcpyDeviceToHost);
    PtCounters &c = sc->counters;
    std::memset(&c, 0, sizeof c);
    c.camera_rays = d.camera_rays; c.intersect_tests = d.intersect_tests; c.shadow_tests = d.shadow_tests;
    c.bvh_nodes_visited = d.nodes; c.triangle_tests = d.tri_tests; c.sphere_tests = d.sphere_tests;
    c.zero_radiance_paths_num = d.zero_num; c.zero_radiance_paths_den = d.zero_den;
    for (int i = 0; i < 16; ++i) c.path_length_hist[i] = d.path_len[i];
    c.sanitized_nan = d.san_nan; c.sanitized_negative = d.san_neg; c.sanitized_infinite = d.san_inf;
    c.film_splats = d.splats; c.wavefront_stages = d.stages; c.reference_asserts = d.ref_asserts;
    for (int k = 0; k < kNumClasses; ++k) for (auto &s : sc->stats) if (s.name == kClasses[k].stat) { s.items = d.shade_items[k]; s.nodes = d.shade_bytes[k]; }
    static const char *kn[5] = {"extend", "extend_mis", "shadow", "extend_camera", "extend_probe"};
    for (int k = 0; k < 5; ++k) for (auto &s : sc->stats) if (s.name == kn[k]) { s.nodes = d.k_nodes[k]; s.tris = d.k_tris[k]; if (k == 4) s.items = d.k_rays[k]; }
    for (auto &s : sc->stats) if (s.name == "trace") { s.nodes = d.k_nodes[0] + d.k_nodes[1] + d.k_nodes[2]; s.tris = d.k_tris[0] + d.k_tris[1] + d.k_tris[2]; }
    if (!g_trace_split) {
        for (int k = 0; k < 3; ++k) if (d.k_rays[k]) { bool have = false; for (auto &s : sc->stats) have = have || s.name == kn[k];
            if (!have) { Stat s2{std::string("trace:") + kn[k]}; s2.items = d.k_rays[k]; s2.nodes = d.k_nodes[k]; s2.tris = d.k_tris[k]; sc->stats.push_back(s2); } }
    }
    for (auto &s : sc->stats) if (s.name == "bssrdf") { s.items = d.bss_items; s.nodes = d.bss_bytes; }
#ifdef PT_TRACE_UTIL
    fprintf(stderr, "[trace-util] kernel saw leaf_quorum = %llu, refill_min = %llu (last launch)\n", d.dbg[0], d.dbg[1]);
    for (int k = 0; k < 4; ++k) if (d.tail[5 + 2 * k])
        fprintf(stderr, "[trace-util] %-14s wave slots busy %.1f %% of launch span x resident waves (the rest: launch ramp + tail after the queue drained)\n", kn[k], 100.0 * (double)d.tail[4 + 2 * k] / (double)d.tail[5 + 2 * k]);
    if (d.tail[2]) fprintf(stderr, "[trace-util] all trace launches: transform step %.3e wave iterations, %.1f %% lanes active, %.1f %% of the waves' cycles; record step (fetch + node / leaf + pop) %.1f %% of the cycles\n",
                           (double)d.tail[12], d.tail[12] ? 100.0 * (double)d.tail[13] / (64.0 * (double)d.tail[12]) : 0.0, 100.0 * (double)d.tail[14] / (double)d.tail[2], 100.0 * (double)d.tail[15] / (double)d.tail[2]);
    if (d.tail[2]) fprintf(stderr, "[trace-util] instance entries tried %.4e, turned away by the object's root test %.4e (%.1f %%), left with a hit %.4e (%.1f %%); stack entries written beyond the LDS ones %.4e\n",
                           (double)d.util2[4], (double)d.util2[5], d.util2[4] ? 100.0 * (double)d.util2[5] / (double)d.util2[4] : 0.0, (double)d.util2[6], d.util2[4] ? 100.0 * (double)d.util2[6] / (double)d.util2[4] : 0.0, (double)d.util2[7]);
    if (d.tail[2]) fprintf(stderr, "[trace-util] record step by part, %% of the waves' cycles: loads issued + waited for %.1f, node branch %.1f, leaf branch %.1f, pops %.1f\n",
                           100.0 * (double)d.util2[0] / (double)d.tail[2], 100.0 * (double)d.util2[1] / (double)d.tail[2], 100.0 * (double)d.util2[2] / (double)d.tail[2], 100.0 * (double)d.util2[3] / (double)d.tail[2]);
    for (int k = 0; k < 4; ++k)
        fprintf(stderr, "[trace-util] %-14s node phase: %.3e wave iterations, %.1f %% lanes active; leaf phase: %.3e iterations, %.1f %% lanes active\n", kn[k], (double)d.regions[4 * k],
                d.regions[4 * k] ? 100.0 * (double)d.regions[4 * k + 1] / (64.0 * (double)d.regions[4 * k]) : 0.0, (double)d.regions[4 * k + 2], d.regions[4 * k + 2] ? 100.0 * (double)d.regions[4 * k + 3] / (64.0 * (double)d.regions[4 * k + 2]) : 0.0);
#endif
#ifdef PT_REGION_PROFILE
    {
        static const char *rn[16] = {"0 loop/queue read", "1 resolve", "2 resolve env le", "3 load ray/hit + fill_hit + Le", "4 sobol window", "5 light choice",
                                     "6 light sample_li", "7 bsdf f/pdf + shadow ray", "8 MIS bsdf sample + store", "9 MIS light pdf_li", "10 bsdf build", "11 continuation sample + RR",
                                     "12 state write-back", "13 queue push/flush", "14 tail", "15 prologue"};
        unsigned long long tot = 0; for (int i = 0; i < 16; ++i) tot += d.regions[i];
        for (int i = 0; i < 16; ++i) fprintf(stderr, "[region] %-34s %6.2f %%  %.3e cycles\n", rn[i], tot ? 100.0 * (double)d.regions[i] / (double)tot : 0.0, (double)d.regions[i]);
    }
#endif
}

int check_spp(const PtRenderParams *rp) { return rp->spp == 0 ? fail(PT_ERR_INVALID_ARG, "spp must be > 0") : PT_OK; }
int check_sample_range(const PtRenderParams *rp, uint32_t first, uint32_t n) {
    if (n == 0) return fail(PT_ERR_INVALID_ARG, "n_samples must be > 0");
    if ((uint64_t)first + n > rp->spp) return fail(PT_ERR_INVALID_ARG, "sample range [" + std::to_string(first) + ", " + std::to_string((uint64_t)first + n) + ") exceeds the job's spp = " + std::to_string(rp->spp));
    return PT_OK;
}
uint32_t tile_slots(const RenderConst &rc) { const uint32_t ntiles = rc.ntx * rc.nty; return rc.tile_rank < ntiles ? (ntiles - rc.tile_rank + rc.tile_world - 1) / rc.tile_world : 0; }

int check_tile_list(const uint32_t *tiles, uint32_t n, uint64_t n_grid, const char *what) {
    if (n > 0 && !tiles) return fail(PT_ERR_INVALID_ARG, std::string(what) + ": null tile list");
    for (uint32_t i = 0; i < n; ++i) {
        if (tiles[i] >= n_grid) return fail(PT_ERR_INVALID_ARG, std::string(what) + ": tile " + std::to_string(tiles[i]) + " is outside the grid of " + std::to_string(n_grid) + " tiles");
        if (i > 0 && tiles[i] <= tiles[i - 1]) return fail(PT_ERR_INVALID_ARG, std::string(what) + ": the tile list must be strictly ascending (entry " + std::to_string(i) + ")");
// ... 198 lines not shown
```

pbrt-rust_amd/csrc/tu_aux.hip:

```cpp
#include "kern_aux.h"
template __global__ void k_shade_miss<false, false>(DeviceScene, RenderConst, PathSoA, ShadeJob);
template __global__ void k_shade_miss<true, false>(DeviceScene, RenderConst, PathSoA, ShadeJob);
template __global__ void k_shade_miss<true, true>(DeviceScene, RenderConst, PathSoA, ShadeJob);
template __global__ void k_film_final<false>(DeviceScene, RenderConst, PathSoA, const float *, float *, DevCounters *);
template __global__ void k_film_final<true>(DeviceScene, RenderConst, PathSoA, const float *, float *, DevCounters *);
```

Baseline: 1992.

## Merge extend, MIS and shadow queues into one tagged ray queue

Shade kernels now push extension, MIS and shadow rays into a single LDS-backed ray queue. Each entry keeps the ray kind in the top two bits of the path id, and one atomic per wave covers all three kinds. The mixed trace kernel reads that one queue and decodes the kind per entry, replacing the prefix-offset lookup across three separate queues. The split-trace mode adds a kernel that separates the queue again, plus an extra host sync. Path capacity is capped at 2^29, and a test entry point checks the new push logic.

```diff
diff --git a/include/mi355pt.h b/include/mi355pt.h
--- a/include/mi355pt.h
+++ b/include/mi355pt.h
@@ -363,6 +363,8 @@
                    float *out_origins, float *out_dirs);
 int pt_dist1d_sample(const float *func, uint32_t n, int discrete, uint32_t n_u, const float *u,
                      float *out_x, float *out_pdf, int32_t *out_offset);
+int pt_test_ray_queue_push(uint32_t qcap, uint32_t n_blocks, uint32_t rounds, const uint8_t *masks,
+                           uint32_t *out_rays, uint32_t *out_n_rays, uint32_t *out_ext, uint32_t *out_n_ext);
 
 #ifdef __cplusplus
 }
diff --git a/pbrt-rust_amd/_abi.py b/pbrt-rust_amd/_abi.py
--- a/pbrt-rust_amd/_abi.py
+++ b/pbrt-rust_amd/_abi.py
@@ -180,6 +180,7 @@
     "pt_halton_samples": (C.c_int, [i32p, u32, u32, i32p, u32p, u32, fp, u64p]),
     "pt_camera_rays": (C.c_int, [C.POINTER(PtRenderParams), u32, fp, fp, fp]),
     "pt_dist1d_sample": (C.c_int, [fp, u32, C.c_int, u32, fp, fp, fp, i32p]),
+    "pt_test_ray_queue_push": (C.c_int, [u32, u32, u32, u8p, u32p, u32p, u32p, u32p]),
 }
 
 
diff --git a/pbrt-rust_amd/csrc/kern_aux.h b/pbrt-rust_amd/csrc/kern_aux.h
--- a/pbrt-rust_amd/csrc/kern_aux.h
+++ b/pbrt-rust_amd/csrc/kern_aux.h
@@ -131,6 +131,19 @@
     (void)zero_num;
 }
 
+template <int QCAP> __global__ __launch_bounds__(256) void k_test_ray_queue(const uint8_t *masks, uint32_t rounds, ShadeJob job) {
+    __shared__ VertexQueues<QCAP, false, false> s_q;
+    s_q.init();
+    __syncthreads();
+    for (uint32_t r = 0; r < rounds; ++r) {
+        const uint32_t t = (blockIdx.x * rounds + r) * 256u + threadIdx.x;
+        const uint32_t m = masks[t];
+        s_q.push(job, t, (m & 1u) != 0u, false, (m & 4u) != 0u, (m & 2u) != 0u);
+        s_q.flush(job, 256u, false);
+    }
+    s_q.flush(job, 0u, true);
+}
+
 template <bool SPH, bool VOL>
 __global__ __launch_bounds__(256, PT_MISS_WAVES) void k_shade_miss(DeviceScene s, RenderConst rc, PathSoA ps, ShadeJob job) {
     __shared__ uint32_t s_hist[16];
diff --git a/pbrt-rust_amd/csrc/kern_decl.h b/pbrt-rust_amd/csrc/kern_decl.h
--- a/pbrt-rust_amd/csrc/kern_decl.h
+++ b/pbrt-rust_amd/csrc/kern_decl.h
@@ -8,10 +8,12 @@
 __global__ void k_medium_route(DeviceScene s, RenderConst rc, SobolTables tabs, PathSoA ps, const uint32_t *queue, const uint32_t *count_ptr,
                                uint32_t *class_count, uint32_t *c0, uint32_t *c1, uint32_t *c2, uint32_t *c3, uint32_t *c4, uint32_t *c5, uint32_t *error);
 __global__ void k_shade_medium(DeviceScene s, RenderConst rc, SobolTables tabs, LightGrid grid, PathSoA ps, ShadeJob job);
+template <int QCAP> __global__ void k_test_ray_queue(const uint8_t *masks, uint32_t rounds, ShadeJob job);
 __global__ void k_build_packets(DeviceScene s, const uint32_t *ordered, uint32_t n_refs, TriPacket *out);
 __global__ void k_mark_leaf_ends(TriPacket *leaf, const uint32_t *last_index, uint32_t n);
 __global__ void k_light_area(DeviceScene s, const uint32_t *head, float *area, float4 *rec);
 template <int NQ, int CAP> __global__ void k_route(DeviceScene s, const uint32_t *queue, const uint32_t *count_ptr, PathSoA ps, uint32_t *class_count, RouteJob rj);
+__global__ void k_split_rays(const uint32_t *rays, const uint32_t *count_ptr, uint32_t *mis, uint32_t *mis_count, uint32_t *shadow, uint32_t *shadow_count);
 __global__ void k_generate(RenderConst rc, SobolTables tabs, PathSoA ps, uint32_t *q_ext, uint32_t *q_ext_count, DevCounters *counters);
 __global__ void k_film(RenderConst rc, PathSoA ps, const float *filter_table, float *film_rgbw, DevCounters *counters);
 template <bool SPH> __global__ void k_film_final(DeviceScene s, RenderConst rc, PathSoA ps, const float *filter_table, float *film_rgbw, DevCounters *counters);
diff --git a/pbrt-rust_amd/csrc/kern_misc.h b/pbrt-rust_amd/csrc/kern_misc.h
--- a/pbrt-rust_amd/csrc/kern_misc.h
+++ b/pbrt-rust_amd/csrc/kern_misc.h
@@ -98,6 +98,24 @@
     }
 #pragma unroll
     for (int k = 0; k < NQ; ++k) if ((uint32_t)k < rj.n_slots) lq_flush_nosync(q[k], class_count + rj.cls_of_slot[k], rj.buf[k], 0u, true);
+}
+__global__ __launch_bounds__(256) void k_split_rays(const uint32_t *rays, const uint32_t *count_ptr, uint32_t *mis, uint32_t *mis_count, uint32_t *shadow, uint32_t *shadow_count) {
+    __shared__ LdsQueue<1024> q_mis, q_sh;
+    lq_init(q_mis); lq_init(q_sh);
+    __syncthreads();
+    const uint32_t count = *count_ptr;
+    const uint32_t rounded = (count + 255u) & ~255u;
+    for (uint32_t qi = blockIdx.x * blockDim.x + threadIdx.x; qi < rounded; qi += gridDim.x * blockDim.x) {
+        const uint32_t e = qi < count ? rays[qi] : 0u;
+        lq_push(q_mis, e & kRayPidMask, (e >> kRayKindShift) == 1u);
+        lq_push(q_sh, e & kRayPidMask, (e >> kRayKindShift) == 2u);
+        __syncthreads();
+        lq_flush_nosync(q_mis, mis_count, mis, 256u, false);
+        lq_flush_nosync(q_sh, shadow_count, shadow, 256u, false);
+        __syncthreads();
+    }
+    lq_flush_nosync(q_mis, mis_count, mis, 0u, true);
+    lq_flush_nosync(q_sh, shadow_count, shadow, 0u, true);
 }
 PT_DEV void camera_ray(const RenderConst &rc, float pfx, float pfy, float time_u, P2 plens_u, V3 &o, V3 &d) {
     V3 pcamera = xf_point(rc.raster_to_camera, V3(pfx, pfy, 0.0f));
diff --git a/pbrt-rust_amd/csrc/kern_shade_common.h b/pbrt-rust_amd/csrc/kern_shade_common.h
--- a/pbrt-rust_amd/csrc/kern_shade_common.h
+++ b/pbrt-rust_amd/csrc/kern_shade_common.h
@@ -150,15 +150,29 @@
 
 
 template <int QCAP, bool PROBE, bool SELF> struct VertexQueues {
-    LdsQueue<QCAP> ext, res, sh, mis;
+    static constexpr int kRayCap = 2 * QCAP > 768 ? 2 * QCAP : 768;
+    LdsQueue<QCAP> ext, res;
+    LdsQueue<kRayCap> rays;
     LdsQueue<PROBE ? QCAP : 1> probe;
     LdsQueue<SELF ? QCAP : 1> self;
-    PT_DEV void init() { lq_init(ext); lq_init(res); lq_init(sh); lq_init(mis); lq_init(probe); lq_init(self); }
+    PT_DEV void init() { lq_init(ext); lq_init(res); lq_init(rays); lq_init(probe); lq_init(self); }
+    PT_DEV void push_rays(uint32_t pid, bool to_ext, bool to_mis, bool to_shadow) {
+        const unsigned long long m_e = __ballot(to_ext), m_m = __ballot(to_mis), m_s = __ballot(to_shadow), any = m_e | m_m | m_s;
+        if (any == 0ull) return;
+        const uint32_t lane = lane_id(), leader = (uint32_t)__ffsll((long long)any) - 1u;
+        const unsigned long long below = (1ull << lane) - 1ull;
+        uint32_t base = 0;
+        if (lane == leader) base = atomicAdd(&rays.count, (uint32_t)(__popcll(m_e) + __popcll(m_m) + __popcll(m_s)));
+        base = __shfl(base, (int)leader);
+        uint32_t at = base + (uint32_t)(__popcll(m_e & below) + __popcll(m_m & below) + __popcll(m_s & below));
+        if (to_ext) rays.buf[at++] = pid;
+        if (to_mis) rays.buf[at++] = pid | (1u << kRayKindShift);
+        if (to_shadow) rays.buf[at] = pid | (2u << kRayKindShift);
+    }
     template <class Job> PT_DEV void push(const Job &job, uint32_t pid, bool to_ext, bool to_resolve, bool to_shadow, bool to_mis, bool to_self = false, bool to_probe = false) {
         lq_push(ext, pid, to_ext);
         lq_push(res, pid, to_resolve && job.shade_next0 != nullptr);
-        lq_push(sh, pid, to_shadow);
-        lq_push(mis, pid, to_mis);
+        push_rays(pid, to_ext, to_mis, to_shadow);
         if constexpr (PROBE) if (job.probe_next) lq_push(probe, pid, to_probe);
         if constexpr (SELF) lq_push(self, pid, to_self);
     }
@@ -166,8 +180,7 @@
         __syncthreads();
         lq_flush_nosync(ext, job.ext_next_count, job.ext_next, reserve, force);
         lq_flush_nosync(res, job.shade_next0_count, job.shade_next0, reserve, force);
-        lq_flush_nosync(sh, job.shadow_count, job.shadow, reserve, force);
-        lq_flush_nosync(mis, job.mis_count, job.mis, reserve, force);
+        lq_flush_nosync(rays, job.rays_count, job.rays, 3u * reserve, force);
         if constexpr (PROBE) if (job.probe_next) lq_flush_nosync(probe, job.probe_next_count, job.probe_next, reserve, force);
         if constexpr (SELF) lq_flush_nosync(self, job.self_next_count, job.self_next, reserve, force);
         __syncthreads();
diff --git a/pbrt-rust_amd/csrc/kern_trace.h b/pbrt-rust_amd/csrc/kern_trace.h
--- a/pbrt-rust_amd/csrc/kern_trace.h
+++ b/pbrt-rust_amd/csrc/kern_trace.h
@@ -69,8 +69,7 @@
     glb_u32 *spill = (glb_u32 *)job.spill + (size_t)(blockIdx.x * (kTraceBlock / 64) + wave_in_block) * 64 * kSpillWords + lane;
     typedef __attribute__((address_space(1))) float glb_f32;
     glb_f32 *wray_g = (glb_f32 *)(spill + (2 * kSpillEntries) * 64);
-    const uint32_t c0 = *job.sub[0].count, c01 = c0 + (MIX ? *job.sub[1].count : 0u);
-    const uint32_t count = c01 + (MIX ? *job.sub[2].count : 0u);
+    const uint32_t count = *job.sub[0].count;
     uint32_t ksel = 0; bool lane_any = ANY == 1;
     __shared__ uint32_t lds_kcnt[MIX ? (kTraceBlock / 64) * 16 : 1];
     uint32_t *kcnt = lds_kcnt + (MIX ? (threadIdx.x >> 6) * 16 : 0u);
@@ -83,10 +82,10 @@
             for (int k = 0; k < 3; ++k) {
                 const TraceSub &S = job.sub[k];
                 uint32_t *r = lds_sub + k * kSubRow;
-                const unsigned long long pq = (unsigned long long)S.queue, pr = (unsigned long long)S.ray, ph = (unsigned long long)S.out_hit, ph2 = (unsigned long long)S.out_hit2,
+                const unsigned long long pr = (unsigned long long)S.ray, ph = (unsigned long long)S.out_hit, ph2 = (unsigned long long)S.out_hit2,
                                          pw = (unsigned long long)S.out_word, pt = (unsigned long long)S.out_t;
-                r[0] = (uint32_t)pq; r[1] = (uint32_t)(pq >> 32); r[2] = (uint32_t)pr; r[3] = (uint32_t)(pr >> 32);
-                r[4] = S.ray_stride; r[5] = (S.per_ray_tmax ? 1u : 0u) | (S.any ? 2u : 0u); r[6] = __float_as_uint(S.scalar_tmax); r[7] = k == 0 ? 0u : (k == 1 ? c0 : c01);
+                r[0] = 0u; r[1] = 0u; r[2] = (uint32_t)pr; r[3] = (uint32_t)(pr >> 32);
+                r[4] = S.ray_stride; r[5] = (S.per_ray_tmax ? 1u : 0u) | (S.any ? 2u : 0u); r[6] = __float_as_uint(S.scalar_tmax); r[7] = 0u;
                 r[8] = (uint32_t)ph; r[9] = (uint32_t)(ph >> 32); r[10] = (uint32_t)ph2; r[11] = (uint32_t)(ph2 >> 32);
                 r[12] = (uint32_t)pw; r[13] = (uint32_t)(pw >> 32); r[14] = (uint32_t)pt; r[15] = (uint32_t)(pt >> 32);
                 r[16] = S.out_hit_stride; r[17] = S.out_word_stride; r[18] = S.out_t_stride; r[19] = 0u;
@@ -264,13 +263,8 @@
             auto load_window = [&](uint32_t base, uint32_t left) {
                 const uint32_t qi = base + lane; uint32_t w = 0u;
                 if (lane < left) {
-                    uint32_t qk = qi; gcu32 *qp = (gcu32 *)PT_SUB(queue);
-                    if constexpr (MIX) {
-                        const uint32_t kk = (qi >= c0 ? 1u : 0u) + (qi >= c01 ? 1u : 0u);
-                        const uint4 r0 = sub_rows[5u * kk], r1 = sub_rows[5u * kk + 1u];
-                        qp = PT_GPTR(const uint32_t, r0.x, r0.y); qk = qi - r1.w;
-                    }
-                    w = qp ? qp[qk] : qk;
+                    gcu32 *qp = (gcu32 *)job.sub[0].queue;
+                    w = qp ? qp[qi] : qi;
                 }
                 return w;
             };
@@ -292,14 +286,13 @@
                 const uint32_t rank = __builtin_amdgcn_mbcnt_hi((uint32_t)(idlem >> 32), __builtin_amdgcn_mbcnt_lo((uint32_t)idlem, 0u));
                 const uint32_t take = min(chunk_left, (uint32_t)__popcll(idlem));
                 const uint32_t wsel = (uint32_t)__shfl((int)qwin, (int)(rank & 63u));
-                const uint32_t qi = chunk_next + rank;
                 get = state == ST_IDLE && rank < take;
                 chunk_next += take; chunk_left -= take;
                 if (get) {
                     gcf4 *rays = (gcf4 *)PT_SUB(ray); uint32_t ray_stride = PT_SUB(ray_stride);
                     pid = wsel;
                     if constexpr (MIX) {
-                        ksel = (qi >= c0 ? 1u : 0u) + (qi >= c01 ? 1u : 0u);
+                        ksel = wsel >> kRayKindShift; pid = wsel & kRayPidMask;
                         const uint4 r0 = sub_rows[5u * ksel], r1 = sub_rows[5u * ksel + 1u];
                         rays = PT_GPTR(const v4f_, r0.z, r0.w);
                         ray_stride = r1.x; per_ray_tmax = (r1.y & 1u) != 0u; lane_any = (r1.y & 2u) != 0u; scalar_tmax = __uint_as_float(r1.z);
diff --git a/pbrt-rust_amd/csrc/kernels.h b/pbrt-rust_amd/csrc/kernels.h
--- a/pbrt-rust_amd/csrc/kernels.h
+++ b/pbrt-rust_amd/csrc/kernels.h
@@ -74,9 +74,13 @@
 constexpr int kBssBytes = 16 * (BssSoA::kProbeQuads + BssSoA::kFrameQuads + BssSoA::kCoefQuads);
 PT_HD bool bss_coef_stored(uint32_t n_textures, const PtMaterial &m) { return n_textures > 0u || m.kd_subsurface != 0u; }
 
+constexpr uint32_t kRayKindShift = 30u, kRayPidMask = (1u << kRayKindShift) - 1u;
+constexpr size_t kMaxRayQueuePaths = (size_t)1 << 29;
+
 struct QueueSet {
     uint32_t *ext[2];
     uint32_t *shade[2][kNumClasses];
+    uint32_t *rays;
     uint32_t *shadow, *mis;
     uint32_t *probe[2];
 };
@@ -84,6 +88,7 @@
     uint32_t ext[2];
     uint32_t shade[2][kNumClasses];
     uint32_t shadow, mis;
+    uint32_t rays;
     uint32_t probe[2];
     uint32_t head[4];
     uint32_t error;
@@ -156,7 +161,7 @@
     const uint32_t *queue; const uint32_t *count;
     uint32_t *ext_next, *ext_next_count;
     uint32_t *shade_next0, *shade_next0_count;
-    uint32_t *shadow, *shadow_count, *mis, *mis_count;
+    uint32_t *rays, *rays_count;
     uint32_t *error;
     DevCounters *counters;
     uint32_t cls;
@@ -169,7 +174,7 @@
     const uint32_t *queue; const uint32_t *count;
     uint32_t *ext_next, *ext_next_count;
     uint32_t *shade_next0, *shade_next0_count;
-    uint32_t *shadow, *shadow_count, *mis, *mis_count;
+    uint32_t *rays, *rays_count;
     uint32_t *error;
     DevCounters *counters;
     BssSoA bs;
diff --git a/pbrt-rust_amd/csrc/parity_api.hip b/pbrt-rust_amd/csrc/parity_api.hip
--- a/pbrt-rust_amd/csrc/parity_api.hip
+++ b/pbrt-rust_amd/csrc/parity_api.hip
@@ -144,4 +144,30 @@
     return PT_OK;
 }
 
+int pt_test_ray_queue_push(uint32_t qcap, uint32_t n_blocks, uint32_t rounds, const uint8_t *masks, uint32_t *out_rays, uint32_t *out_n_rays, uint32_t *out_ext, uint32_t *out_n_ext) {
+    DevTmp scratch;
+    if (!masks || !out_rays || !out_n_rays || !out_ext || !out_n_ext) return fail(PT_ERR_INVALID_ARG, "null argument");
+    if (qcap != 256u && qcap != (uint32_t)PT_P2_QCAP && qcap != 1024u) return fail(PT_ERR_INVALID_ARG, "qcap: 256, " + std::to_string(PT_P2_QCAP) + " or 1024 (the shade kernels' LDS queue sizes)");
+    const size_t n = (size_t)n_blocks * rounds * 256;
+    if (n == 0 || n > kRayPidMask) return fail(PT_ERR_INVALID_ARG, "n_blocks * rounds * 256 must be in [1, 2^30)");
+    int st = ensure_device();
+    if (st) return st;
+    uint8_t *dmasks; uint32_t *drays, *dext, *dcount;
+    HIP_TRY(scratch.alloc(&dmasks, n)); HIP_TRY(scratch.alloc(&drays, 3 * n * 4)); HIP_TRY(scratch.alloc(&dext, n * 4)); HIP_TRY(scratch.alloc(&dcount, 8));
+    HIP_TRY(hipMemcpy(dmasks, masks, n, hipMemcpyHostToDevice));
+    HIP_TRY(hipMemset(dcount, 0, 8));
+    ShadeJob job{}; job.rays = drays; job.rays_count = dcount; job.ext_next = dext; job.ext_next_count = dcount + 1;
+    if (qcap == 256u) hipLaunchKernelGGL(k_test_ray_queue<256>, dim3(n_blocks), dim3(256), 0, 0, dmasks, rounds, job);
+    else if (qcap == 1024u) hipLaunchKernelGGL(k_test_ray_queue<1024>, dim3(n_blocks), dim3(256), 0, 0, dmasks, rounds, job);
+    else hipLaunchKernelGGL(k_test_ray_queue<PT_P2_QCAP>, dim3(n_blocks), dim3(256), 0, 0, dmasks, rounds, job);
+    HIP_TRY(hipDeviceSynchronize());
+    uint32_t cnt[2];
+    HIP_TRY(hipMemcpy(cnt, dcount, 8, hipMemcpyDeviceToHost));
+    if (cnt[0] > 3 * n || cnt[1] > n) return fail(PT_ERR_HIP, "ray queue test: more entries than were pushed");
+    HIP_TRY(hipMemcpy(out_rays, drays, (size_t)cnt[0] * 4, hipMemcpyDeviceToHost));
+    HIP_TRY(hipMemcpy(out_ext, dext, (size_t)cnt[1] * 4, hipMemcpyDeviceToHost));
+    *out_n_rays = cnt[0]; *out_n_ext = cnt[1];
+    return PT_OK;
 }
+
+}
diff --git a/pbrt-rust_amd/csrc/render_loop.hip b/pbrt-rust_amd/csrc/render_loop.hip
--- a/pbrt-rust_amd/csrc/render_loop.hip
+++ b/pbrt-rust_amd/csrc/render_loop.hip
@@ -65,7 +65,7 @@
 static int shaded_in(const pt_scene *sc, int c, bool volpath) { return !sc->class_used[c] ? -1 : !volpath ? c : c == kSpecClass ? 1 : (int)class_general((uint32_t)c); }
 static bool class_launched(const pt_scene *sc, int q, bool volpath) { for (int c = 0; c < kNumClasses; ++c) if (shaded_in(sc, c, volpath) == q) return true; return false; }
 static bool class_has_queue(const pt_scene *sc, int c) { return c == 0 || kClasses[c].kind != kSurface || class_launched(sc, c, false) || class_launched(sc, c, true); }
-static size_t n_queues(const pt_scene *sc) { size_t n = 2 + 2 + (sc->has_bssrdf ? 2 : 0); for (int c = 0; c < kNumClasses; ++c) n += class_has_queue(sc, c) ? 2 : 0; return n; }
+static size_t n_queues(const pt_scene *sc) { size_t n = 2 + 3 + (g_trace_split ? 2 : 0) + (sc->has_bssrdf ? 2 : 0); for (int c = 0; c < kNumClasses; ++c) n += class_has_queue(sc, c) ? 2 : 0; return n; }
 
 int launch_trace(pt_scene *sc, int any, TraceJob job, uint32_t n_upper, bool probe) {
     if (n_upper == 0) return PT_OK;
@@ -123,12 +123,15 @@
             float4 *bp = (float4 *)sc->bss_slab;
             bs.probe = bp; bp += capacity * (size_t)BssSoA::kProbeQuads; bs.frame = bp; bp += capacity * (size_t)BssSoA::kFrameQuads; bs.coef = bp;
         }
+        if (capacity > kMaxRayQueuePaths) { drop(); return fail(PT_ERR_INVALID_ARG, "more than 2^29 paths in one pass: a ray-queue entry keeps the path id beside the ray's kind"); }
         e = hipMalloc((void **)&sc->qbuf, n_queues(sc) * capacity * 4);
         if (e != hipSuccess) { sc->qbuf = nullptr; return oom("queues", e); }
         uint32_t *qp = sc->qbuf;
         for (int i = 0; i < 2; ++i) { sc->q.ext[i] = qp; qp += capacity; }
         for (int i = 0; i < 2; ++i) for (int c = 0; c < kNumClasses; ++c) { sc->q.shade[i][c] = nullptr; if (class_has_queue(sc, c)) { sc->q.shade[i][c] = qp; qp += capacity; } }
-        sc->q.shadow = qp; qp += capacity; sc->q.mis = qp; qp += capacity;
+        sc->q.rays = qp; qp += 3 * capacity;
+        sc->q.shadow = sc->q.mis = nullptr;
+        if (g_trace_split) { sc->q.shadow = qp; qp += capacity; sc->q.mis = qp; qp += capacity; }
         sc->q.probe[0] = sc->q.probe[1] = nullptr;
         if (sc->has_bssrdf) { sc->q.probe[0] = qp; qp += capacity; sc->q.probe[1] = qp; }
         sc->capacity = capacity;
@@ -296,7 +299,7 @@
     if (threadIdx.x != 0 || blockIdx.x != 0) return;
     int nxt = 1 - cur;
     if (mask & 1u) { qc->ext[nxt] = 0; qc->probe[nxt] = 0; for (int c = 0; c < kNumClasses; ++c) qc->shade[nxt][c] = 0; }
-    if (mask & 2u) { qc->shadow = 0; qc->mis = 0; }
+    if (mask & 2u) { qc->rays = 0; qc->shadow = 0; qc->mis = 0; }
     if (mask & 4u) { for (int i = 0; i < 4; ++i) qc->head[i] = 0; }
     if (mask & 8u) { qc->ext[cur] = 0; qc->probe[cur] = 0; for (int c = 0; c < kNumClasses; ++c) qc->shade[cur][c] = 0; }
 }
@@ -366,7 +369,7 @@
     return PT_OK;
 }
 
-struct Iter { pt_scene *sc; const RenderConst &rc; const LightGrid &grid; bool fin, profile_exact; int index, cur; uint32_t n_ext, n_resolve, n_shadow, n_mis, n_probe, n_stage_b; };
+struct Iter { pt_scene *sc; const RenderConst &rc; const LightGrid &grid; bool fin, profile_exact; int index, cur; uint32_t n_ext, n_resolve, n_rays, n_probe, n_stage_b; };
 
 template <class Job> Job shading_job(const Iter &it, const uint32_t *queue, const uint32_t *count, int self) {
     pt_scene *sc = it.sc; QCounters *qc = sc->qc; const int nxt = 1 - it.cur;
@@ -374,7 +377,7 @@
     j.ext_next = sc->q.ext[nxt]; j.ext_next_count = &qc->ext[nxt];
     if (!it.fin) { j.shade_next0 = sc->q.shade[nxt][kMissClass]; j.shade_next0_count = &qc->shade[nxt][kMissClass]; }
     j.self_next = sc->q.shade[nxt][self]; j.self_next_count = &qc->shade[nxt][self];
-    j.shadow = sc->q.shadow; j.shadow_count = &qc->shadow; j.mis = sc->q.mis; j.mis_count = &qc->mis;
+    j.rays = sc->q.rays; j.rays_count = &qc->rays;
     j.error = &qc->error; j.counters = sc->dc;
     return j;
 }
@@ -401,15 +404,23 @@
     TraceSub sh = trace_sub(sc->q.shadow, &qc->shadow, ps.nee, PathSoA::kNeeWords, 1.0f - 0.0001f, 2);
     sh.out_word = &ps.occluded(0); sh.out_word_stride = PathSoA::kNeeWords; sh.any = rc.volpath ? 0u : 1u;
     if (shells) { sh.out_hit = (float4 *)ps.ext + 4; sh.out_hit_stride = PathSoA::kExtWords / 4; sh.out_hit2 = (float4 *)ps.ext + 5; }
-    if (it.n_mis + it.n_shadow == 0 || g_trace_split) {
+    if (it.n_rays == it.n_ext || g_trace_split) {
         auto one = [&](const char *stat, const TraceSub &sub, int head, int any, uint32_t n) { TraceJob tj = trace_job(sc, head); tj.sub[0] = sub; return traced(sc, stat, any, tj, n); };
         int st;
-        if ((st = one(it.index == 0 ? "extend_camera" : "extend", ext, 0, 0, it.n_ext)) || (st = one("extend_mis", mis, 1, 0, it.n_mis))) return st;
-        return one("shadow", sh, 2, (int)sh.any, it.n_shadow);
+        uint32_t n_mis = 0, n_shadow = 0;
+        if (it.n_rays != it.n_ext) {
+            hipLaunchKernelGGL(k_split_rays, blocks_for(it.n_rays, 8u), dim3(256), 0, sc->stream, (const uint32_t *)sc->q.rays, (const uint32_t *)&qc->rays, sc->q.mis, &qc->mis, sc->q.shadow, &qc->shadow);
+            QCounters h;
+            if ((st = sync_queue_counters(sc, h))) return st;
+            n_mis = h.mis; n_shadow = h.shadow;
+        }
+        if ((st = one(it.index == 0 ? "extend_camera" : "extend", ext, 0, 0, it.n_ext)) || (st = one("extend_mis", mis, 1, 0, n_mis))) return st;
+        return one("shadow", sh, 2, (int)sh.any, n_shadow);
     }
     TraceJob tj = trace_job(sc, 0);
     tj.sub[0] = ext; tj.sub[1] = mis; tj.sub[2] = sh;
-    return traced(sc, "trace", 2, tj, it.n_ext + it.n_mis + it.n_shadow);
+    tj.sub[0].queue = sc->q.rays; tj.sub[0].count = &qc->rays;
+    return traced(sc, "trace", 2, tj, it.n_rays);
 }
 
 static void route_hits(const Iter &it) {
@@ -495,14 +506,14 @@
         if (it.index == max_iterations) return fail(PT_ERR_PROBE_CHAIN, "pass did not finish within " + std::to_string(max_iterations) + " wavefront iterations");
         const int cur = it.cur;
         if (debug_iter && it.index > 0 && it.index % 2048 == 0) {
-            fprintf(stderr, "[iter %d] ext %u shadow %u mis %u probe %u shade:", it.index, h.ext[cur], h.shadow, h.mis, h.probe[cur]);
+            fprintf(stderr, "[iter %d] ext %u rays %u probe %u shade:", it.index, h.ext[cur], h.rays, h.probe[cur]);
             for (int c = 0; c < kNumClasses; ++c) fprintf(stderr, " %u", h.shade[cur][c]);
             fprintf(stderr, "\n");
         }
-        it.n_ext = h.ext[cur]; it.n_resolve = h.shade[cur][kMissClass]; it.n_shadow = h.shadow; it.n_mis = h.mis; it.n_probe = h.probe[cur];
+        it.n_ext = h.ext[cur]; it.n_resolve = h.shade[cur][kMissClass]; it.n_rays = it.index == 0 ? h.ext[cur] : h.rays; it.n_probe = h.probe[cur];
         it.n_stage_b = 0;
         if (rc.volpath && (sc->ds.has_grid || sc->ds.has_shells)) for (int c = 0; c < kNumClasses; ++c) if (c != kMissClass) it.n_stage_b += h.shade[cur][c];
-        if (it.n_ext == 0 && it.n_resolve == 0 && it.n_probe == 0 && it.n_stage_b == 0 && (!it.fin || (it.n_shadow == 0 && it.n_mis == 0))) break;
+        if (it.n_ext == 0 && it.n_resolve == 0 && it.n_probe == 0 && it.n_stage_b == 0 && (!it.fin || it.n_rays == 0)) break;
         reset(4u | 1u);
         if ((st = trace_rays(it))) return st;
         route_hits(it);
diff --git a/pbrt-rust_amd/csrc/tu_aux.hip b/pbrt-rust_amd/csrc/tu_aux.hip
--- a/pbrt-rust_amd/csrc/tu_aux.hip
+++ b/pbrt-rust_amd/csrc/tu_aux.hip
@@ -2,5 +2,8 @@
 template __global__ void k_shade_miss<false, false>(DeviceScene, RenderConst, PathSoA, ShadeJob);
 template __global__ void k_shade_miss<true, false>(DeviceScene, RenderConst, PathSoA, ShadeJob);
 template __global__ void k_shade_miss<true, true>(DeviceScene, RenderConst, PathSoA, ShadeJob);
+template __global__ void k_test_ray_queue<256>(const uint8_t *, uint32_t, ShadeJob);
+template __global__ void k_test_ray_queue<PT_P2_QCAP>(const uint8_t *, uint32_t, ShadeJob);
+template __global__ void k_test_ray_queue<1024>(const uint8_t *, uint32_t, ShadeJob);
 template __global__ void k_film_final<false>(DeviceScene, RenderConst, PathSoA, const float *, float *, DevCounters *);
 template __global__ void k_film_final<true>(DeviceScene, RenderConst, PathSoA, const float *, float *, DevCounters *);
```

Result: faster. 2034, median of 6 (+2.1%).
